# jxx2/MetaFEM.jl

Measured on AMD Instinct MI355X. Metric: DOF-updates/sec (assembly+CG iter) on 3D hex thermal conduction, higher is better.
Workload: dtype f64; 1 GPU; 3D thermal conduction, linear hex-8, 512x512x512 structured mesh (make_Brick): fused assembly (K + R) + 200 Jacobi-CG iterations per step; n_dof=135005697, nnz=3630961153, parallelism=single GPU

## Files before the change

include/metafem_mi355x_debug.h:

```cpp
#ifndef METAFEM_MI355X_DEBUG_H
#define METAFEM_MI355X_DEBUG_H

#include "metafem_mi355x.h"

#ifdef __cplusplus
extern "C" {
#endif

int64_t mfem_debug_sym_spmv_count(void);
long long mfem_debug_symp_fingerprint_count(void);
long long mfem_debug_symp_coded_count(void);
long long mfem_debug_symp_trim_count(void);
long long mfem_debug_symp_const_count(void);
long long mfem_debug_symp_const_steps(void);
int mfem_debug_spmv_scaled_layout(mfem_context ctx, mfem_csr A, const double* vals, const double* ssym, const double* x, double* y, double alpha, double beta,
                                  const double* dotw, double* partials_out , int32_t cap, int32_t* n_partials , int32_t* form );
int mfem_debug_set(const char* key, int64_t a, int64_t b);

int mfem_debug_lat27_cg_fused(void);
int64_t mfem_debug_lat27_pass1_bytes(mfem_csr A);
long long mfem_debug_lat27_spmv_count(void);
double mfem_debug_lat27_asymmetry(mfem_csr A);
long long mfem_debug_lat8_spmv_count(void);
double mfem_debug_lat8_asymmetry(mfem_csr A);
int mfem_debug_graph_comm_count(void);
long long mfem_debug_graph_launch_count(void);
int64_t mfem_debug_mesh_rows_count(void);
int64_t mfem_debug_mesh_direct_count(void);
int64_t mfem_debug_ws_bytes(mfem_context ctx);
int64_t mfem_debug_mesh_residual_count(void);
int64_t mfem_debug_mesh_operator_count(void);
int64_t mfem_debug_brick_operator_count(void);
int mfem_debug_brick_operator_apply_dot(mfem_context ctx, uint64_t op, const double* x, double* y, double alpha, double beta, const double* dotw,
                                        double* partials, int32_t* n_partials );
int64_t mfem_debug_mesh_ops_count(void);
int64_t mfem_debug_mesh_variants(int32_t reset);
int64_t mfem_debug_op_wave_count(int32_t kernel);
int64_t mfem_debug_sell_periodic_blocks(mfem_csr A);
int64_t mfem_debug_hex27_rows_count(void);
int64_t mfem_debug_hex27_mixed_count(void);
int64_t mfem_debug_hex27_direct_count(void);
int mfem_prof_spmv_enable(mfem_context ctx, int on);
int mfem_prof_spmv_read(mfem_context ctx, double* total_ms , int64_t* launches , int reset);
int mfem_prof_comm_enable(mfem_context ctx, int on);
int mfem_prof_comm_read(mfem_context ctx, double* halo_wait_ms , int64_t* halo_waits , double* allreduce_ms ,
                        int64_t* allreduces , int reset);
int mfem_debug_comm_selftest(mfem_context ctx, int64_t count, int32_t rounds);

unsigned long long mfem_debug_ws_address(mfem_context ctx);
long long mfem_debug_cg_ring_count(void);

int mfem_debug_ws_trial_log(mfem_context ctx, double* out4);

int mfem_debug_fail_host_alloc(int nth);


int mfem_debug_bsell_fields(mfem_csr A);
long long mfem_debug_bsell_spmv_count(void);
int mfem_debug_remainder_info(mfem_csr A, int64_t* rows , int64_t* entries , double* asym_before );
long long mfem_debug_rem_spmv_count(void);
int mfem_debug_csr_tplan(mfem_csr A, int64_t* bytes , double* build_ms );
int mfem_debug_brick_operator_signed_diagonal(mfem_context ctx, uint64_t op, double* d);
int mfem_debug_brick_multigrid_transfer(mfem_context ctx, uint64_t mg, int32_t level, int32_t restriction, const double* in, double* out);
double* mfem_debug_brick_multigrid_coords(uint64_t mg, int32_t level, int32_t dim_id);

#ifdef __cplusplus
}
#endif
#endif
```

metafem.jl_amd/_lib.py:

```python
from __future__ import annotations

import ctypes as C
import os

import torch

_HERE = os.path.dirname(os.path.abspath(__file__))
LIB_PATH = os.path.join(_HERE, "libmetafem_mi355x.so")


class MetaFEMError(RuntimeError):
    pass


def _load():
    if not os.path.exists(LIB_PATH):
        raise ImportError(
            f"{LIB_PATH} is missing: build it with `python -c 'import __graft_entry__ as g; g.build()'` "
            "(or `make -C metafem.jl_amd/csrc`).  There is no CPU fallback.")
    return C.CDLL(LIB_PATH, mode=C.RTLD_GLOBAL)


class _Lib:

    def __init__(self, cdll):
        object.__setattr__(self, "_cdll", cdll)

    def __getattr__(self, name):
        if name.startswith("mfem_debug_set_"):
            key = name[len("mfem_debug_set_"):]
            cdll = self._cdll

            def knob(a=0, b=0, _key=key):
                if _key == "recheck_scale":
                    return cdll.mfem_debug_set(b"recheck_scale_ppm", int(round(float(a) * 1e6)), 0)
                return cdll.mfem_debug_set(_key.encode(), int(a), int(b))
            return knob
        return getattr(self._cdll, name)


lib = _Lib(_load())

c_void_p, c_int, c_int32, c_int64, c_double, c_uint64, c_uint32 = (
    C.c_void_p, C.c_int, C.c_int32, C.c_int64, C.c_double, C.c_uint64, C.c_uint32)


class SolveOptions(C.Structure):
    _fields_ = [("method", c_int32), ("precond", c_int32), ("l_or_s", c_int32), ("maxiter", c_int32),
                ("max_pass", c_int32), ("check_every", c_int32), ("converge_tol", c_double), ("seed", c_uint64),
                ("fixed_iterations", c_int32), ("scale_in_place", c_int32), ("left_precond", c_int32),
                ("cg_variant", c_int32)]


class SolveStats(C.Structure):
    _fields_ = [("passes", c_int32), ("iterations", c_int32), ("final_res", c_double), ("initial_res", c_double),
                ("solve_ms", c_double), ("converged", c_int32), ("spmv_count", c_int32)]


class ThermalParams(C.Structure):
    _fields_ = [("k", c_double), ("h", c_double), ("Tenv", c_double), ("robin_faces", c_uint32), ("fixed_faces", c_uint32),
                ("h_penalty", c_double), ("Tw", c_double)]


class ElasticityParams(C.Structure):
    _fields_ = [("lam", c_double), ("mu", c_double), ("tau", c_double), ("penalty_faces", c_uint32),
                ("traction_faces", c_uint32), ("sig", c_double * 6)]


class KvalTerm(C.Structure):
    _fields_ = [("dual_sd", c_int32), ("base_sd", c_int32), ("block", c_int32), ("reserved", c_int32)]


class ResBatchTerm(C.Structure):
    _fields_ = [("dual_sd", c_int32), ("reserved", c_int32), ("cpID_shift", c_int64)]


class VarBatchTerm(C.Structure):
    _fields_ = [("sd", c_int32), ("reserved", c_int32), ("cpID_shift", c_int64), ("x", C.c_void_p)]


class ConstTerm(C.Structure):
    _fields_ = [("dual_sd", c_int32), ("base_sd", c_int32), ("block", c_int32), ("reserved", c_int32), ("coef", c_double)]


MAX_BATCH_TERMS = 48


class MeshDirectStats(C.Structure):
    _fields_ = [(n, c_int64) for n in ("batches", "tasks", "max_batch_doubles", "max_batch_elements", "geometry_evaluations", "device_bytes",
                                       "waves_per_trip", "max_control_point_doubles", "budget_doubles", "waves_per_workgroup", "lds_bytes",
                                       "split_owners", "max_batch_owners")]


class ResSymbol(C.Structure):
    _fields_ = [("word", c_int32), ("reserved", c_int32), ("shift", c_int64), ("x", C.c_void_p)]


class AffineTerm(C.Structure):
    _fields_ = [("dual_pos", c_int32), ("dual_sd", c_int32), ("n_pairs", c_int32), ("reserved", c_int32), ("c0", c_double),
                ("sym", c_int32 * 8), ("normal", c_int32 * 8), ("coef", c_double * 8)]


MAX_RES_SYMBOLS, MAX_RES_TERMS, MAX_RES_PAIRS = 16, 48, 8


class OperatorTerm(C.Structure):
    _fields_ = [("dual_sd", c_int32), ("base_sd", c_int32), ("block", c_int32), ("reserved", c_int32), ("coef", c_double),
                ("normal_coef", c_double * 3)]


MG_MAX_LEVELS = 12


class MultigridOptions(C.Structure):
    _fields_ = [("smoother_degree", c_int32), ("coarse_degree", c_int32), ("smoothing_range", c_double), ("coarse_range", c_double),
                ("eig_steps", c_int32), ("max_levels", c_int32)]


class MultigridInfo(C.Structure):
    _fields_ = [("levels", c_int32), ("sign", c_int32), ("nx", c_int32 * 12), ("ny", c_int32 * 12), ("nz", c_int32 * 12),
                ("lambda_max", c_double * 12), ("products", c_int64 * 12), ("setup_products", c_int64), ("bytes", c_int64), ("cycles", c_int64),
                ("setups", c_int64)]


ALLREDUCE_CB = C.CFUNCTYPE(c_int, c_void_p, C.POINTER(c_double), c_int32)
EXCHANGE_CB = C.CFUNCTYPE(c_int, c_void_p, C.POINTER(c_double), C.POINTER(c_double), C.POINTER(c_double), C.POINTER(c_double), c_int64)


class CommHostOps(C.Structure):
    _fields_ = [("user", c_void_p), ("allreduce_sum", ALLREDUCE_CB), ("neighbour_exchange", EXCHANGE_CB), ("flags", c_uint32),
                ("reserved", c_uint32)]


COMM_HOST_POISON_GHOSTS = 1


class OpLayout(C.Structure):
    _fields_ = [("itg", c_int32), ("itp", c_int32), ("n_sd", c_int32), ("n_host", c_int64), ("index_base", c_int32),
                ("n_colours", c_int32), ("colour_offsets", C.POINTER(c_int64))]


P = c_void_p
SIGNATURES = {
    "mfem_abi_version": (c_int, []),
    "mfem_last_error": (C.c_char_p, []),
    "mfem_context_create": (c_int, [c_int, P, C.POINTER(P)]),
    "mfem_context_set_stream": (c_int, [P, P]),
    "mfem_context_destroy": (c_int, [P]),
    "mfem_context_sync": (c_int, [P]),
    "mfem_csr_create": (c_int, [P, c_int64, c_int64, P, c_int, P, c_int, C.POINTER(P)]),
    "mfem_csr_destroy": (c_int, [P]),
    "mfem_spmv_csr": (c_int, [P, P, P, P, P, c_double, c_double]),
    "mfem_spmv_csr_t": (c_int, [P, P, P, P, P, c_double, c_double]),
    "mfem_axpby": (c_int, [P, c_int64, c_double, P, c_double, P]),
    "mfem_dot": (c_int, [P, c_int64, P, P, C.POINTER(c_double)]),
    "mfem_nrm2": (c_int, [P, c_int64, P, C.POINTER(c_double)]),
    "mfem_rand": (c_int, [P, c_int64, c_uint64, c_uint32, P]),
    "mfem_jacobi_by_diagonal": (c_int, [P, P, P, P]),
    "mfem_jacobi2_by_column": (c_int, [P, P, P, P]),
    "mfem_jacobi_by_row": (c_int, [P, P, P, P]),
    "mfem_mat_div_jacobi": (c_int, [P, P, P, P]),
    "mfem_debug_hex27_direct_count": (c_int64, []),
    "mfem_debug_hex27_mixed_count": (c_int64, []),
    "mfem_debug_hex27_rows_count": (c_int64, []),
    "mfem_debug_mesh_rows_count": (c_int64, []),
    "mfem_debug_mesh_variants": (c_int64, [c_int32]),
    "mfem_debug_op_wave_count": (c_int64, [c_int32]),
    "mfem_debug_bsell_fields": (c_int, [P]),
    "mfem_debug_bsell_spmv_count": (c_int64, []),
    "mfem_debug_sell_periodic_blocks": (c_int64, [P]),
    "mfem_debug_symp_fingerprint_count": (C.c_longlong, []),
    "mfem_debug_symp_coded_count": (C.c_longlong, []),
    "mfem_debug_symp_trim_count": (C.c_longlong, []),
    "mfem_debug_symp_const_count": (C.c_longlong, []),
    "mfem_debug_symp_const_steps": (C.c_longlong, []),
    "mfem_debug_spmv_scaled_layout": (c_int, [P, P, P, P, P, P, c_double, c_double, P, P, c_int32, C.POINTER(c_int32), C.POINTER(c_int32)]),
    "mfem_debug_set": (c_int, [C.c_char_p, c_int64, c_int64]),
    "mfem_debug_graph_comm_count": (c_int, []),
    "mfem_debug_graph_launch_count": (C.c_longlong, []),
    "mfem_debug_cg_ring_count": (C.c_longlong, []),
    "mfem_debug_lat27_cg_fused": (c_int, []),
    "mfem_debug_lat27_pass1_bytes": (c_int64, [P]),
    "mfem_prof_spmv_enable": (c_int, [P, c_int]),
    "mfem_prof_spmv_read": (c_int, [P, C.POINTER(c_double), C.POINTER(c_int64), c_int]),
    "mfem_prof_comm_enable": (c_int, [P, c_int]),
    "mfem_prof_comm_read": (c_int, [P, C.POINTER(c_double), C.POINTER(c_int64), C.POINTER(c_double), C.POINTER(c_int64), c_int]),
    "mfem_solve": (c_int, [P, P, P, P, P, C.POINTER(SolveOptions), C.POINTER(SolveStats)]),
    "mfem_solve_set_shadow": (c_int, [P, P, c_int32]),
    "mfem_brick_create": (c_int, [P, c_int32, c_int32, c_int32, c_double, c_double, c_double, c_int32, c_int32,
                                  C.POINTER(P)]),
    "mfem_brick_destroy": (c_int, [P]),
    "mfem_brick_num_controlpoints": (c_int64, [P]),
    "mfem_brick_num_elements": (c_int64, [P]),
    "mfem_brick_coords": (P, [P, c_int32]),
    "mfem_brick_set_slab": (c_int, [P, c_int32, c_int32]),
    "mfem_brick_pattern": (c_int, [P, P, c_int32, C.POINTER(P)]),
    "mfem_pattern_build": (c_int, [P, c_int32, c_int64, c_int64, P, c_int32, c_int32, C.POINTER(P), P]),
    "mfem_csr_rowptr64": (P, [P]),
    "mfem_csr_colidx": (P, [P]),
    "mfem_csr_nnz": (c_int64, [P]),
    "mfem_csr_n": (c_int64, [P]),
    "mfem_brick_assemble_thermal": (c_int, [P, P, P, C.POINTER(ThermalParams), P]),
    "mfem_brick_residual_thermal": (c_int, [P, P, C.POINTER(ThermalParams), P, P, P]),
    "mfem_brick_assemble_elasticity": (c_int, [P, P, P, C.POINTER(ElasticityParams), P]),
    "mfem_brick_residual_elasticity": (c_int, [P, P, C.POINTER(ElasticityParams), P, P]),
    "mfem_update_basic_elements": (c_int, [P, c_int32, c_int32, c_int32, c_int64, c_int64, P, P, P, P, c_int32, P, P]),
    "mfem_update_basic_boundary": (c_int, [P, c_int32, c_int32, c_int32, c_int32, c_int64, c_int64, P, P, P, P, P, P, P,
                                          c_int32, P, P, P]),
    "mfem_op_var": (c_int, [P, C.POINTER(OpLayout), P, c_int32, c_int64, P, P, P, P, P, c_int64]),
    "mfem_op_kval": (c_int, [P, C.POINTER(OpLayout), P, c_int32, c_int32, P, P, c_int64, P, P, P, c_int64]),
    "mfem_op_res": (c_int, [P, C.POINTER(OpLayout), P, c_int32, P, c_int64, P, P, P, P, c_int64]),
    "mfem_debug_lat27_spmv_count": (c_int64, []),
    "mfem_debug_lat27_asymmetry": (C.c_double, [c_void_p]),
    "mfem_debug_lat8_spmv_count": (c_int64, []),
    "mfem_debug_lat8_asymmetry": (C.c_double, [c_void_p]),
    "mfem_spmv_solver_layout": (c_int, [P, P, P, P, P, c_double, c_double]),
    "mfem_spmv_solver_layout_dot": (c_int, [P, P, P, P, P, c_double, c_double, C.POINTER(c_double)]),
    "mfem_csr_solver_layout": (c_int, [P, P, C.POINTER(c_int32), C.POINTER(c_int32), C.POINTER(c_int64), C.POINTER(c_int64)]),
    "mfem_csr_solver_layout_entries": (c_int, [P, P, C.POINTER(c_int64), C.POINTER(c_int32)]),
    "mfem_csr_solver_layout_bytes": (c_int, [P, P, C.POINTER(c_int64)]),
    "mfem_debug_sym_spmv_count": (c_int64, []),
    "mfem_op_kval_batch": (c_int, [P, C.POINTER(OpLayout), P, c_int32, C.POINTER(KvalTerm), P, P, c_int64, c_int64, P, P, P, c_int64]),
    "mfem_op_res_batch": (c_int, [P, C.POINTER(OpLayout), P, c_int32, C.POINTER(ResBatchTerm), P, P, P, P, P, c_int64]),
    "mfem_op_var_batch": (c_int, [P, C.POINTER(OpLayout), P, c_int32, C.POINTER(VarBatchTerm), P, P, P, P, c_int64]),
    "mfem_mesh_assemble_elements": (c_int, [P, c_int32, c_int32, c_int32, c_int64, c_int64, P, P, P, P, c_int32, c_int32,
                                            C.POINTER(ConstTerm), P, c_int64, P, P, c_int64, c_int32, C.POINTER(c_int64)]),
    "mfem_mesh_assemble_elements_rows": (c_int, [P, c_int32, c_int32, c_int32, c_int64, c_int64, P, P, P, P, c_int32, c_int32,
                                                 C.POINTER(ConstTerm), c_int32, P, P, P, P, P]),
    "mfem_mesh_assemble_elements_rows_set": (c_int, [P, c_int32, c_int32, c_int32, c_int64, c_int64, P, P, P, P, c_int32, c_int32,
                                                 C.POINTER(ConstTerm), c_int32, P, P, P, P, P]),
    "mfem_mesh_direct_plan_create": (c_int, [P, c_int32, c_int64, c_int64, c_int32, P, P, P, P, c_int32, P, C.POINTER(c_uint64)]),
    "mfem_mesh_direct_plan_destroy": (c_int, [c_uint64]),
    "mfem_mesh_direct_plan_stats": (c_int, [c_uint64, C.POINTER(MeshDirectStats)]),
    "mfem_mesh_assemble_elements_direct": (c_int, [P, c_int32, c_int32, c_int32, c_int64, c_int64, P, P, P, P, c_int32, c_int32,
                                                   C.POINTER(ConstTerm), c_int32, P, c_uint64, P, c_int32]),
    "mfem_debug_mesh_direct_count": (c_int64, []),
    "mfem_debug_ws_bytes": (c_int64, [P]),
    "mfem_mesh_row_ranks": (c_int, [P, c_int32, c_int64, c_int64, c_int32, P, P, P, P, c_int32, P]),
    "mfem_mesh_assemble_facets": (c_int, [P, c_int32, c_int32, c_int32, c_int32, c_int64, c_int64, P, P, P, P, P, P, P, c_int32,
                                          c_int32, C.POINTER(ConstTerm), P, c_int64, P, P, c_int64, c_int32, C.POINTER(c_int64)]),
    "mfem_mesh_residual_elements": (c_int, [P, c_int32, c_int32, c_int32, c_int64, c_int64, P, P, P, P, c_int32, c_int32,
                                            C.POINTER(ResSymbol), c_int32, C.POINTER(AffineTerm), P, P, P]),
    "mfem_mesh_residual_facets": (c_int, [P, c_int32, c_int32, c_int32, c_int32, c_int64, c_int64, P, P, P, P, P, P, P, c_int32,
                                          c_int32, C.POINTER(ResSymbol), c_int32, C.POINTER(AffineTerm), P, P, P]),
    "mfem_debug_mesh_residual_count": (c_int64, []),
    "mfem_mesh_operator_create": (c_int, [P, c_int32, c_int32, c_int64, c_int64, c_int32, P, P, c_int32, C.POINTER(c_uint64)]),
    "mfem_mesh_operator_set_elements": (c_int, [c_uint64, c_int32, P, P, P, P, c_int32, C.POINTER(OperatorTerm)]),
    "mfem_mesh_operator_add_facets": (c_int, [c_uint64, c_int32, c_int32, c_int64, P, P, P, P, P, P, P, c_int32, C.POINTER(OperatorTerm),
                                              C.POINTER(c_int32)]),
    "mfem_mesh_operator_set_terms": (c_int, [c_uint64, c_int32, c_int32, C.POINTER(OperatorTerm)]),
    "mfem_mesh_operator_set_variable_terms": (c_int, [c_uint64, c_int32, c_int32, C.POINTER(KvalTerm), P]),
    "mfem_mesh_operator_destroy": (c_int, [c_uint64]),
    "mfem_mesh_operator_apply": (c_int, [P, c_uint64, P, P, c_double, c_double]),
    "mfem_mesh_operator_diagonal": (c_int, [P, c_uint64, P]),
    "mfem_solve_operator": (c_int, [P, c_uint64, P, P, C.POINTER(SolveOptions), C.POINTER(SolveStats)]),
    "mfem_debug_mesh_operator_count": (c_int64, []),
    "mfem_brick_operator_create": (c_int, [P, P, C.POINTER(ThermalParams), C.POINTER(c_uint64)]),
    "mfem_brick_operator_set_params": (c_int, [c_uint64, C.POINTER(ThermalParams)]),
    "mfem_brick_operator_create_elasticity": (c_int, [P, P, C.POINTER(ElasticityParams), C.POINTER(c_uint64)]),
    "mfem_brick_operator_set_elasticity_params": (c_int, [c_uint64, C.POINTER(ElasticityParams)]),
    "mfem_brick_operator_create_hex27": (c_int, [P, P, C.POINTER(ThermalParams), C.POINTER(c_uint64)]),
    "mfem_brick_operator_destroy": (c_int, [c_uint64]),
    "mfem_brick_operator_apply": (c_int, [P, c_uint64, P, P, c_double, c_double]),
    "mfem_brick_operator_diagonal": (c_int, [P, c_uint64, P]),
    "mfem_debug_brick_operator_count": (c_int64, []),
    "mfem_debug_brick_operator_signed_diagonal": (c_int, [P, c_uint64, P]),
    "mfem_debug_brick_operator_apply_dot": (c_int, [P, c_uint64, P, P, c_double, c_double, P, P, C.POINTER(c_int32)]),
    "mfem_brick_multigrid_create": (c_int, [P, c_uint64, C.POINTER(MultigridOptions), C.POINTER(c_uint64)]),
    "mfem_brick_multigrid_create_elasticity": (c_int, [P, c_uint64, C.POINTER(MultigridOptions), C.POINTER(c_uint64)]),
    "mfem_brick_multigrid_create_hex27": (c_int, [P, c_uint64, C.POINTER(MultigridOptions), C.POINTER(c_uint64)]),
    "mfem_brick_multigrid_setup": (c_int, [P, c_uint64]),
    "mfem_brick_multigrid_apply": (c_int, [P, c_uint64, P, P]),
    "mfem_brick_multigrid_info": (c_int, [c_uint64, C.POINTER(MultigridInfo)]),
    "mfem_brick_multigrid_destroy": (c_int, [c_uint64]),
    "mfem_debug_brick_multigrid_transfer": (c_int, [P, c_uint64, c_int32, c_int32, P, P]),
    "mfem_debug_brick_multigrid_coords": (P, [c_uint64, c_int32, c_int32]),
    "mfem_mesh_var_elements": (c_int, [P, c_int32, c_int32, c_int32, c_int64, c_int64, P, P, P, P, c_int32, c_int32,
                                       C.POINTER(VarBatchTerm), P, P, c_int64]),
    "mfem_mesh_var_facets": (c_int, [P, c_int32, c_int32, c_int32, c_int32, c_int64, c_int64, P, P, P, P, P, P, P, c_int32,
                                     c_int32, C.POINTER(VarBatchTerm), P, P, P, c_int64]),
    "mfem_mesh_res_elements": (c_int, [P, c_int32, c_int32, c_int32, c_int64, c_int64, P, P, P, P, c_int32, c_int32,
                                       C.POINTER(ResBatchTerm), P, P, P, P, P]),
    "mfem_mesh_res_facets": (c_int, [P, c_int32, c_int32, c_int32, c_int32, c_int64, c_int64, P, P, P, P, P, P, P, c_int32,
                                     c_int32, C.POINTER(ResBatchTerm), P, P, P, P, P]),
    "mfem_mesh_kval_elements": (c_int, [P, c_int32, c_int32, c_int32, c_int64, c_int64, P, P, P, P, c_int32, c_int32,
                                        C.POINTER(KvalTerm), P, P, c_int64, P, P, c_int64, c_int32, C.POINTER(c_int64)]),
    "mfem_mesh_kval_elements_rows": (c_int, [P, c_int32, c_int32, c_int32, c_int64, c_int64, P, P, P, P, c_int32, c_int32,
                                             C.POINTER(KvalTerm), P, P, c_int32, P, P, P, P, P]),
    "mfem_mesh_kval_facets": (c_int, [P, c_int32, c_int32, c_int32, c_int32, c_int64, c_int64, P, P, P, P, P, P, P, c_int32,
                                      c_int32, C.POINTER(KvalTerm), P, P, c_int64, P, P, c_int64, c_int32, C.POINTER(c_int64)]),
    "mfem_debug_mesh_ops_count": (c_int64, []),
    "mfem_comm_unique_id": (c_int, [P]),
    "mfem_comm_create": (c_int, [P, c_int32, c_int32, P, C.POINTER(P)]),
    "mfem_comm_destroy": (c_int, [P]),
    "mfem_context_set_comm": (c_int, [P, P, c_int64, c_int64, c_int32]),
    "mfem_allreduce_sum": (c_int, [P, P, c_int32]),
    "mfem_halo_exchange": (c_int, [P, P]),
    "mfem_halo_reduce": (c_int, [P, P]),
    "mfem_comm_create_host": (c_int, [P, c_int32, c_int32, C.POINTER(CommHostOps), C.POINTER(P)]),
    "mfem_csr_ncols": (c_int64, [P]),
    "mfem_csr_replan": (c_int, [P, P]),
    "mfem_csr_spmv_bytes": (c_int, [P, P, C.POINTER(c_int64), C.POINTER(c_int64)]),
    "mfem_debug_comm_selftest": (c_int, [P, c_int64, c_int32]),
    "mfem_debug_ws_address": (C.c_ulonglong, [P]),
    "mfem_debug_fail_host_alloc": (c_int, [c_int]),
    "mfem_debug_ws_trial_log": (c_int, [P, C.POINTER(C.c_double)]),
    "mfem_debug_remainder_info": (c_int, [P, C.POINTER(c_int64), C.POINTER(c_int64), C.POINTER(C.c_double)]),
    "mfem_debug_rem_spmv_count": (C.c_longlong, []),
    "mfem_debug_csr_tplan": (c_int, [P, C.POINTER(c_int64), C.POINTER(C.c_double)]),
}

for _name, (_res, _args) in SIGNATURES.items():
    _fn = getattr(lib, _name)
    _fn.restype = _res
    _fn.argtypes = _args


def check(rc: int) -> None:
    if rc != 0:
        raise MetaFEMError(f"libmetafem_mi355x rc={rc}: {lib.mfem_last_error().decode()}")
```

metafem.jl_amd/csrc/api.hip:

```cpp
#include <stdarg.h>
#include <atomic>

#include <exception>
#include <mutex>
#include <new>
#include <set>

#include "common.h"
#include <string>

static std::mutex g_ctx_mutex;
static std::set<mfem_context_s*> g_live_contexts;
bool mfem_context_alive(mfem_context_s* ctx) {
  std::lock_guard<std::mutex> lk(g_ctx_mutex);
  return g_live_contexts.count(ctx) != 0;
}

static thread_local char g_err[1024] = "";

void mfem_set_error(const char* fmt, ...) {
  va_list ap;
  va_start(ap, fmt);
  vsnprintf(g_err, sizeof(g_err), fmt, ap);
  va_end(ap);
}

int mfem_api_exception(const char* entry) noexcept {
  try {
    throw;
  } catch (const std::bad_alloc&) {
    mfem_set_error("%s: host memory exhausted (std::bad_alloc)", entry);
    return MFEM_ERR_ALLOC;
  } catch (const std::exception& e) {
    mfem_set_error("%s: internal error: %s", entry, e.what());
    return MFEM_ERR_INTERNAL;
  } catch (...) {
    mfem_set_error("%s: internal error (unknown C++ exception)", entry);
    return MFEM_ERR_INTERNAL;
  }
}

static std::atomic<int> g_fail_host_alloc{0};
extern "C" int mfem_debug_fail_host_alloc(int nth) try {
  g_fail_host_alloc.store(nth > 0 ? nth : 0);
  return MFEM_OK;
} MFEM_API_CATCH("mfem_debug_fail_host_alloc")
void mfem_host_alloc_probe() {
  int v = g_fail_host_alloc.load();
  while (v > 0) {
    if (g_fail_host_alloc.compare_exchange_weak(v, v - 1)) {
      if (v == 1) throw std::bad_alloc();
      return;
    }
  }
}

std::atomic<int> mfem_debug_epoch{0};

extern "C" int mfem_abi_version(void) { return MFEM_ABI_VERSION; }
extern "C" const char* mfem_last_error(void) { return g_err; }

int mfem_ws_release(void* raw);
static int context_allocate(mfem_context_s* c) {
  MFEM_CHECK_HIP(hipMalloc(&c->d_partials, sizeof(double) * MFEM_MAX_PARTIALS * 8));
  MFEM_CHECK_HIP(hipMalloc(&c->d_scalars, sizeof(double) * MFEM_NSCALARS));
  MFEM_CHECK_HIP(hipHostMalloc(&c->h_scalars, sizeof(double) * MFEM_NSCALARS));
  MFEM_CHECK_HIP(hipMalloc(&c->d_flags, sizeof(int32_t) * MFEM_NFLAGS));
  MFEM_CHECK_HIP(hipHostMalloc(&c->h_flags, sizeof(int32_t) * MFEM_NFLAGS));
  MFEM_CHECK_HIP(hipMemsetAsync(c->d_scalars, 0, sizeof(double) * MFEM_NSCALARS, c->stream));
  MFEM_CHECK_HIP(hipMemsetAsync(c->d_flags, 0, sizeof(int32_t) * MFEM_NFLAGS, c->stream));
  MFEM_CHECK_HIP(hipEventCreate(&c->ev0));
  MFEM_CHECK_HIP(hipEventCreate(&c->ev1));
  return MFEM_OK;
}

static void context_release(mfem_context_s* ctx) {
  if (ctx->d_partials) hipFree(ctx->d_partials);
  if (ctx->d_scalars) hipFree(ctx->d_scalars);
  if (ctx->h_scalars) hipHostFree(ctx->h_scalars);
  if (ctx->d_flags) hipFree(ctx->d_flags);
  if (ctx->h_flags) hipHostFree(ctx->h_flags);
  (void)mfem_ws_release(ctx->ws_raw);
  (void)mfem_ws_release(ctx->ws_alt_raw);
  if (ctx->prof_ev) {
    for (int i = 0; i < 2 * MFEM_PROF_PAIRS; ++i)
      if (ctx->prof_ev[i]) hipEventDestroy(ctx->prof_ev[i]);
    delete[] ctx->prof_ev;
  }
  if (ctx->ev0) hipEventDestroy(ctx->ev0);
  if (ctx->ev1) hipEventDestroy(ctx->ev1);
  for (int i = 0; i < MFEM_GRAPH_SLOTS; ++i)
    if (ctx->graph_exec[i]) hipGraphExecDestroy(ctx->graph_exec[i]);
  if (ctx->graph_ev) hipEventDestroy(ctx->graph_ev);
  if (ctx->graph_stream) hipStreamDestroy(ctx->graph_stream);
}

extern "C" int mfem_context_create(int device, void* stream, mfem_context* out) try {
  MFEM_REQUIRE(out != nullptr, "out is null");
  int ndev = 0;
  MFEM_CHECK_HIP(hipGetDeviceCount(&ndev));
  MFEM_REQUIRE(device >= 0 && device < ndev, "no such HIP device");
  MFEM_CHECK_HIP(hipSetDevice(device));
  hipDeviceProp_t prop;
  MFEM_CHECK_HIP(hipGetDeviceProperties(&prop, device));
  if (strncmp(prop.gcnArchName, "gfx950", 6) != 0) {
    mfem_set_error("libmetafem_mi355x is built for gfx950 only, device %d is %s", device, prop.gcnArchName);
    return MFEM_ERR_UNSUPPORTED;
  }
  mfem_host_alloc_probe();
  mfem_context_s* c = new mfem_context_s();
  memset(c, 0, sizeof(*c));
  c->device = device;
  c->stream = (hipStream_t)stream;
  c->num_cus = prop.multiProcessorCount;
  int rc = context_allocate(c);
  if (rc != MFEM_OK) {
    context_release(c);
    delete c;
    return rc;
  }
  {
    std::lock_guard<std::mutex> lk(g_ctx_mutex);
    g_live_contexts.insert(c);
  }
  *out = c;
  return MFEM_OK;
} MFEM_API_CATCH("mfem_context_create")

extern "C" int mfem_context_set_stream(mfem_context ctx, void* stream) try {
  MFEM_REQUIRE(ctx != nullptr, "ctx is null");
  ctx->stream = (hipStream_t)stream;
  return MFEM_OK;
} MFEM_API_CATCH("mfem_context_set_stream")

extern "C" int mfem_context_sync(mfem_context ctx) try {
  MFEM_REQUIRE(ctx != nullptr, "ctx is null");
  MFEM_CHECK_HIP(hipStreamSynchronize(ctx->stream));
  return MFEM_OK;
} MFEM_API_CATCH("mfem_context_sync")

extern "C" int mfem_context_destroy(mfem_context ctx) try {
  if (!ctx) return MFEM_OK;
  {
    std::lock_guard<std::mutex> lk(g_ctx_mutex);
    g_live_contexts.erase(ctx);
  }
  hipStreamSynchronize(ctx->stream);
  context_release(ctx);
  delete ctx;
  return MFEM_OK;
} MFEM_API_CATCH("mfem_context_destroy")

int mfem_prof_flush(mfem_context_s* ctx) {
  if (ctx->prof_used == 0) return MFEM_OK;
  MFEM_CHECK_HIP(hipEventSynchronize(ctx->prof_ev[2 * ctx->prof_used - 1]));
  for (int k = 0; k < ctx->prof_used; ++k) {
    float ms = 0.f;
    MFEM_CHECK_HIP(hipEventElapsedTime(&ms, ctx->prof_ev[2 * k], ctx->prof_ev[2 * k + 1]));
    ctx->prof_ms += ms;
  }
  ctx->prof_count += ctx->prof_used;
  ctx->prof_used = 0;
  return MFEM_OK;
}

extern "C" int mfem_prof_spmv_enable(mfem_context ctx, int on) try {
  MFEM_REQUIRE(ctx, "null ctx");
  if (on && !ctx->prof_ev) {
    ctx->prof_ev = new hipEvent_t[2 * MFEM_PROF_PAIRS]();
    for (int i = 0; i < 2 * MFEM_PROF_PAIRS; ++i) MFEM_CHECK_HIP(hipEventCreate(&ctx->prof_ev[i]));
  }
  if (!on) {
    int rc = mfem_prof_flush(ctx);
    if (rc) return rc;
  }
  ctx->prof_on = on ? 1 : 0;
  return MFEM_OK;
} MFEM_API_CATCH("mfem_prof_spmv_enable")

extern "C" int mfem_prof_spmv_read(mfem_context ctx, double* total_ms, int64_t* launches, int reset) try {
  MFEM_REQUIRE(ctx && total_ms && launches, "null argument");
  int rc = mfem_prof_flush(ctx);
  if (rc) return rc;
  *total_ms = ctx->prof_ms;
  *launches = ctx->prof_count;
  if (reset) {
    ctx->prof_ms = 0.0;
    ctx->prof_count = 0;
  }
  return MFEM_OK;
} MFEM_API_CATCH("mfem_prof_spmv_read")

uint64_t mfem_next_csr_serial() {
  static std::atomic<uint64_t> next{1};
  return next.fetch_add(1);
}

void mfem_graphs_invalidate(mfem_context_s* ctx) {
  for (int i = 0; i < MFEM_GRAPH_SLOTS; ++i)
    if (ctx->graph_exec[i]) {
      hipGraphExecDestroy(ctx->graph_exec[i]);
      ctx->graph_exec[i] = nullptr;
      ctx->graph_key[i] = 0;
    }
}

static std::atomic<size_t> g_ws_align{0}, g_ws_offset{0};
extern "C" int mfem_debug_set_ws_placement(long long align, long long offset) try {
  g_ws_align = align > 0 ? (size_t)align : 0;
  g_ws_offset = offset > 0 ? (size_t)offset : 0;
  return MFEM_OK;
} MFEM_API_CATCH("mfem_debug_set_ws_placement")
static int ws_alloc(mfem_context_s* ctx, void** raw, size_t bytes) {
  (void)ctx;
  *raw = nullptr;
  MFEM_CHECK_HIP(hipMalloc(raw, bytes));
  return MFEM_OK;
}
static int ws_free(void* raw) {
  if (raw) MFEM_CHECK_HIP(hipFree(raw));
  return MFEM_OK;
}
int mfem_ws_release(void* raw) { return ws_free(raw); }
extern "C" int64_t mfem_debug_ws_bytes(mfem_context ctx) { return ctx ? (int64_t)ctx->ws_bytes : 0; }
extern "C" unsigned long long mfem_debug_ws_address(mfem_context ctx) { return ctx ? (unsigned long long)(uintptr_t)ctx->ws : 0ull; }
#include <chrono>
static double now_ms() { return std::chrono::duration<double, std::milli>(std::chrono::steady_clock::now().time_since_epoch()).count(); }
int mfem_ws_next_candidate(mfem_context_s* ctx) {
  const bool verbose = getenv("MFEM_WS_TRIAL_VERBOSE") != nullptr;
  double t0 = now_ms();
  MFEM_CHECK_HIP(hipStreamSynchronize(ctx->stream));
  if (verbose) fprintf(stderr, "ws trial: sync %.1f ms\n", now_ms() - t0);
  const size_t need = ctx->ws_bytes + g_ws_align + g_ws_offset;
  if (ctx->ws_alt_raw) {
    t0 = now_ms();
    {
      int rcf = ws_free(ctx->ws_raw);
      if (rcf) return rcf;
    }
    if (verbose) fprintf(stderr, "ws trial: free %.1f ms\n", now_ms() - t0);
    ctx->ws = ctx->ws_raw = nullptr;
  }
  size_t freeb = 0, totalb = 0;
  void* raw = nullptr;
  bool ok = hipMemGetInfo(&freeb, &totalb) == hipSuccess && freeb >= need + ((size_t)4 << 30);
  t0 = now_ms();
  if (ok && ws_alloc(ctx, &raw, need) != MFEM_OK) ok = false;
  if (verbose) fprintf(stderr, "ws trial: alloc %.1f ms\n", now_ms() - t0);
  if (!ok) {
    (void)hipGetLastError();
    if (!ctx->ws_raw) {
      ctx->ws = ctx->ws_alt;
      ctx->ws_raw = ctx->ws_alt_raw;
      ctx->ws_alt = ctx->ws_alt_raw = nullptr;
    }
    return MFEM_OK;
  }
  if (ctx->ws_raw) {
    ctx->ws_alt = ctx->ws;
    ctx->ws_alt_raw = ctx->ws_raw;
  }
  ctx->ws_raw = raw;
  uintptr_t p = (uintptr_t)raw;
  if (g_ws_align) p = (p + g_ws_align - 1) / g_ws_align * g_ws_align;
  ctx->ws = (void*)(p + g_ws_offset);
  ctx->ws_try += 1;
  return MFEM_OK;
}
int mfem_ws_decide(mfem_context_s* ctx, bool keep_current) {
  MFEM_CHECK_HIP(hipStreamSynchronize(ctx->stream));
  if (ctx->ws_alt_raw) {
    if (keep_current) {
      int rcf = ws_free(ctx->ws_alt_raw);
      if (rcf) return rcf;
    } else {
      int rcf = ws_free(ctx->ws_raw);
      if (rcf) return rcf;
      ctx->ws = ctx->ws_alt;
      ctx->ws_raw = ctx->ws_alt_raw;
    }
  }
  ctx->ws_alt = ctx->ws_alt_raw = nullptr;
  ctx->ws_try = 99;
  return MFEM_OK;
}
int mfem_ws_reserve(mfem_context_s* ctx, size_t bytes) {
  if (bytes <= ctx->ws_bytes) return MFEM_OK;
  MFEM_CHECK_HIP(hipStreamSynchronize(ctx->stream));
  int rcf = ws_free(ctx->ws_raw);
  if (!rcf) rcf = ws_free(ctx->ws_alt_raw);
  ctx->ws = ctx->ws_raw = ctx->ws_alt = ctx->ws_alt_raw = nullptr;
  ctx->ws_try = 0;
  ctx->ws_bytes = 0;
  if (rcf) return rcf;
  rcf = ws_alloc(ctx, &ctx->ws_raw, bytes + g_ws_align + g_ws_offset);
  if (rcf) return rcf;
  uintptr_t p = (uintptr_t)ctx->ws_raw;
  if (g_ws_align) p = (p + g_ws_align - 1) / g_ws_align * g_ws_align;
  ctx->ws = (void*)(p + g_ws_offset);
  ctx->ws_bytes = bytes;
  return MFEM_OK;
}

extern "C" {
int mfem_debug_set_spmv(int, int);
int mfem_debug_set_ell(int);
int mfem_debug_set_sell(int);
int mfem_debug_set_lat27(int);
int mfem_debug_set_lat8(int);
int mfem_debug_set_layout_min_rows(int64_t, int64_t);
int mfem_debug_set_graphs(int, int64_t);
int mfem_debug_set_idrs(int);
int mfem_debug_set_bicgstabl(int);
int mfem_debug_set_gmres(int);
int mfem_debug_set_vec_grid(int);
int mfem_debug_set_halo_overlap(int);
int mfem_debug_set_hex27(int);
int mfem_debug_set_elasticity(int);
int mfem_debug_set_hex8_thermal(int);
int mfem_debug_set_ws_placement(long long, long long);
int mfem_debug_set_ws_trial(int);
int mfem_debug_set_cg_streaming(int);
int mfem_debug_set_cg_ring(int);
int mfem_debug_set_cg_single_max_rows(int64_t);
int mfem_debug_set_csr_strips(int, int64_t);
int mfem_debug_set_remainder(int);
int mfem_debug_set_recheck_scale(double);
int mfem_debug_set_bsell(int);
}
extern int g_mesh_gather_rows, g_mesh_abl, g_mesh_stage_min_itp, g_mesh_term_matrix;
extern int g_op_wave_forms, g_op_wave_min_itp;
extern int64_t g_mesh_direct_budget;
extern "C" int mfem_debug_set(const char* key, int64_t a, int64_t b) try {
  MFEM_REQUIRE(key, "null key");
  const std::string k(key);
  if (k == "spmv") return mfem_debug_set_spmv((int)a, (int)b);
  if (k == "ell") return mfem_debug_set_ell((int)a);
  if (k == "sell") return mfem_debug_set_sell((int)a);
  if (k == "lat27") return mfem_debug_set_lat27((int)a);
  if (k == "lat8") return mfem_debug_set_lat8((int)a);
  if (k == "layout_min_rows") return mfem_debug_set_layout_min_rows(a, b);
  if (k == "graphs") return mfem_debug_set_graphs((int)a, b);
  if (k == "idrs") return mfem_debug_set_idrs((int)a);
  if (k == "bicgstabl") return mfem_debug_set_bicgstabl((int)a);
  if (k == "gmres") return mfem_debug_set_gmres((int)a);
  if (k == "vec_grid") return mfem_debug_set_vec_grid((int)a);
  if (k == "halo_overlap") return mfem_debug_set_halo_overlap((int)a);
  if (k == "hex27") return mfem_debug_set_hex27((int)a);
  if (k == "elasticity") return mfem_debug_set_elasticity((int)a);
  if (k == "hex8_thermal") return mfem_debug_set_hex8_thermal((int)a);
  if (k == "ws_placement") return mfem_debug_set_ws_placement((long long)a, (long long)b);
  if (k == "ws_trial") return mfem_debug_set_ws_trial((int)a);
  if (k == "cg_streaming") return mfem_debug_set_cg_streaming((int)a);
  if (k == "cg_ring") return mfem_debug_set_cg_ring((int)a);
  if (k == "cg_single_max_rows") return mfem_debug_set_cg_single_max_rows(a);
  if (k == "csr_strips") return mfem_debug_set_csr_strips((int)a, b);
  if (k == "remainder") return mfem_debug_set_remainder((int)a);
  if (k == "mesh_gather_rows") { g_mesh_gather_rows = (int)a; return MFEM_OK; }
  if (k == "bsell") return mfem_debug_set_bsell((int)a);
  if (k == "op_wave_forms") { g_op_wave_forms = (int)a; g_op_wave_min_itp = b > 0 ? (int)b : 10; return MFEM_OK; }
  if (k == "mesh_stage_min_itp") { g_mesh_stage_min_itp = a > 0 ? (int)a : 16; return MFEM_OK; }
  if (k == "mesh_term_matrix") { g_mesh_term_matrix = (int)a; return MFEM_OK; }
  if (k == "mesh_direct_budget") { g_mesh_direct_budget = a > 0 ? a : 0; return MFEM_OK; }
  if (k == "mesh_abl") { g_mesh_abl = (int)a; return MFEM_OK; }
  if (k == "recheck_scale_ppm") return mfem_debug_set_recheck_scale((double)a * 1e-6);
  mfem_set_error("mfem_debug_set: unknown key '%s'", key);
  return MFEM_ERR_INVALID;
} MFEM_API_CATCH("mfem_debug_set")
```

metafem.jl_amd/csrc/common.h:

```cpp
#pragma once
#include <hip/hip_runtime.h>
#include <atomic>
#include <mutex>
#include <unordered_map>
#include <stdint.h>
#include <stdio.h>
#include <string.h>

#if defined(__HIP_DEVICE_COMPILE__) && !defined(__gfx950__)
#error "metafem_mi355x is written for gfx950 (MI355X) only: counted s_waitcnt vmcnt(k) pipelines assume loads and stores share one in-order counter, global_load_lds_dwordx4 and v_mfma_f64 are used directly -- build with --offload-arch=gfx950"
#endif
#include "../../include/metafem_mi355x.h"
#include "../../include/metafem_mi355x_debug.h"
#include "csr_decide.h"
#include "sell_decide.h"
#include "lat_decide.h"

#define MFEM_WAVE 64
#define MFEM_BLOCK 256
#define MFEM_MAX_PARTIALS 4096
static_assert(LAT_MAX_GATHER_GRID == MFEM_MAX_PARTIALS, "a workgroup of the tiles' gather pass writes one partial sum");
#define MFEM_NFLAGS 80
#define MFEM_NSCALARS 4096

void mfem_set_error(const char* fmt, ...);

int mfem_api_exception(const char* entry) noexcept;
#define MFEM_API_CATCH(entry) catch (...) { return mfem_api_exception(entry); }
void mfem_host_alloc_probe();

#define MFEM_CHECK_HIP(expr)                                                                  \
  do {                                                                                        \
    hipError_t _e = (expr);                                                                   \
    if (_e != hipSuccess) {                                                                   \
      mfem_set_error("%s:%d: %s -> %s", __FILE__, __LINE__, #expr, hipGetErrorString(_e));    \
      return MFEM_ERR_HIP;                                                                    \
    }                                                                                         \
  } while (0)

#define MFEM_REQUIRE(cond, msg)                                      \
  do {                                                               \
    if (!(cond)) {                                                   \
      mfem_set_error("%s:%d: %s (%s)", __FILE__, __LINE__, msg, #cond); \
      return MFEM_ERR_INVALID;                                       \
    }                                                                \
  } while (0)

#define MFEM_CHECK_LAUNCH() MFEM_CHECK_HIP(hipGetLastError())

template <typename T> struct __attribute__((visibility("hidden"))) DevBuf {
  T* p = nullptr;
  DevBuf() = default;
  DevBuf(DevBuf&& o) noexcept : p(o.release()) {}
  DevBuf& operator=(DevBuf&& o) noexcept { if (this != &o) { reset(); p = o.release(); } return *this; }
  DevBuf(const DevBuf&) = delete;
  DevBuf& operator=(const DevBuf&) = delete;
  ~DevBuf() { reset(); }
  hipError_t alloc(size_t count) { reset(); return hipMalloc((void**)&p, sizeof(T) * count); }
  void reset() { if (p) (void)hipFree(p); p = nullptr; }
  T* release() { T* q = p; p = nullptr; return q; }
  operator T*() const { return p; }
};

struct mfem_comm_s;

#define MFEM_MAX_ZONES 8
struct SpmvPart {
  int part;
  int nz;
  int64_t lo[MFEM_MAX_ZONES], hi[MFEM_MAX_ZONES];
};
__host__ __device__ __forceinline__ bool spmv_part_skip(const SpmvPart& P, int64_t r0, int64_t r1) {
  if (P.part == 0) return false;
  bool bnd = false;
  for (int z = 0; z < P.nz; ++z) bnd = bnd || (r0 < P.hi[z] && r1 > P.lo[z]);
  return P.part == 1 ? bnd : !bnd;
}


#define MFEM_GRAPH_SLOTS 4
struct mfem_context_s {
  int device;
  hipStream_t stream;
  int num_cus;
  double* d_partials;
  double* d_scalars;
  double* h_scalars;
  int32_t* d_flags;
  int32_t* h_flags;
  void* ws;
  void* ws_raw;
  size_t ws_bytes;
  int ws_try;
  void* ws_alt;
  void* ws_alt_raw;
  float ws_try_ms;
  float ws_log[4];
  const double* shadow;
  int32_t shadow_count;
  mfem_comm_s* comm;
  int64_t halo_plane_len;
  int32_t halo_fields;
  hipEvent_t ev0, ev1;
  int prof_on;
  int prof_used;
  hipEvent_t* prof_ev;
  double prof_ms;
  int64_t prof_count;
  hipGraphExec_t graph_exec[MFEM_GRAPH_SLOTS];
  uint64_t graph_key[MFEM_GRAPH_SLOTS];
  int graph_next;
  hipStream_t graph_stream;
  hipEvent_t graph_ev;
  int graph_active;
  int force_csr;
  int probe_active;
};
#define MFEM_PROF_PAIRS 1024
int mfem_prof_flush(mfem_context_s* ctx);

struct mfem_operator_head;
struct mfem_csr_s {
  mfem_context_s* ctx;
  uint64_t serial;
  int64_t n, nnz;
  const void* rowptr;
  int rowptr_bits;
  const int32_t* colidx;
  int index_base;
  int32_t max_row_nnz;
  CsrPlan plan;
  int nb_F, nb_checked;
  int64_t rb_ntiles;
  int64_t rb_elided;
  int32_t* rb_rows;
  uint8_t* cw_elide;
  int32_t lat_m1, lat_m2, lat_fields;
  int32_t lat_m0, lat_plo, lat_gw;
  int32_t lat_inferred;
  uint16_t* diag_off;
  void* owned_rowptr;
  void* owned_colidx;
  int64_t x_offset;
  int64_t ncols;
  int ell_state, ell_K;
  int64_t ell_npad;
  int32_t* ell_cols;
  const double* ell_src;
  double* ell_vals;
  int dia_state, dia_classes;
  void* dia_dev;
  int32_t* dia_flags;
  int32_t dia_regular_blocks;
  int dia_triples;
  int sym_state;
  int64_t sym_c0, sym_c1;
  int sym_cls;
  int sym_S;
  int64_t sym_mx, sym_myz;
  int ell_bound_mode;
  int dia_kernel;
  int symp_state;
  int symp_m1, symp_m2;
  int64_t symp_PL;
  int symp_p0, symp_p1;
  int symp_NS, symp_NPk;
  int symp_B;
  int symp_trim;
  int symp_DC;
  int symp_dneg;
  int symp_CS;
  int symp_cs_last;
  int64_t symp_flagged, symp_flagged_last;
  double symp_cst[27];
  int symp_ccode;
  int symp_dc_last;
  double* symp_vals;
  SellLayout sell;
  LatTiles lat27, lat8;
  int lat_refused;
  int rem_active;
  int64_t rem_nrows, rem_nent, rem_cap_rows, rem_cap_ent;
  int32_t* rem_rows;
  int64_t* rem_ptr;
  int32_t* rem_len;
  int32_t* rem_col;
  double* rem_val;
  unsigned long long* rem_cnt;
  void* rem_sort_tmp;
  size_t rem_sort_bytes;
  double rem_asym_before;
  int64_t rem_last_rows, rem_last_ent;
  struct mfem_tplan_s* tplan;
  struct mfem_operator_head* op;
  double* op_scratch;
  const double* op_dsc;
  uint64_t op_epoch;
};
struct mfem_tplan_s {
  mfem_csr_s* AT;
  void* perm;
  int perm_bits;
  double* vals;
  int64_t bytes;
  double build_ms;
};
static inline CsrShape mfem_csr_shape(const mfem_csr_s* A) { return {A->n, A->nnz, A->max_row_nnz}; }
template <typename F> static inline auto mfem_by_rowptr(const mfem_csr_s* A, F&& f) { return A->rowptr_bits == 64 ? f(int64_t{}) : f(int32_t{}); }
int mfem_tplan_get(mfem_context_s* ctx, mfem_csr_s* A, mfem_tplan_s** out);
void mfem_tplan_free(mfem_csr_s* A);
int mfem_tplan_gather(mfem_context_s* ctx, const mfem_tplan_s* P, const double* src, double* valsT, const double* d1, const double* d2);
bool mfem_rem_enabled();
bool mfem_rem_diag();
void mfem_rem_clear(mfem_csr_s* A);
void mfem_rem_free(mfem_csr_s* A);
int mfem_rem_build(mfem_context_s* ctx, mfem_csr_s* A, const double* vals, int n_fields, const double* y1, const double* y2, const double* scale,
                   double gate, bool* built);
int mfem_rem_apply(mfem_context_s* ctx, mfem_csr_s* A, const double* x, const double* dsc, double* y, double alpha, const double* dotw,
                   double* partials, int* n_partials, const int32_t* done_flag);
int64_t mfem_rem_design_bytes(const mfem_csr_s* A);
int mfem_spmv_lat8_launch(mfem_context_s* ctx, mfem_csr_s* A, const double* vals, const double* x, double* y, double alpha, double beta,
                          const double* dotw, double* partials, int* n_partials, const int32_t* done_flag, int part);
int64_t mfem_lat8_design_bytes(const mfem_csr_s* A);
int64_t mfem_lat8_entries(const mfem_csr_s* A);
int mfem_lattice_hint_from_row0(mfem_context_s* ctx, mfem_csr_s* A);
static inline LatShape mfem_lat_shape(const mfem_csr_s* A, int64_t min_rows) {
  return {A->n, A->ncols, A->max_row_nnz, A->lat_m0, A->lat_m1, A->lat_m2, A->lat_fields, A->lat_plo, A->lat_gw, min_rows};
}
static inline void mfem_lat_unbind(mfem_csr_s* A, LatTiles& T) {
  if (T.vals) A->rem_active = 0;
  T.vals = T.dump = nullptr;
  T.src = T.dsc = nullptr;
}
int mfem_sym_probe(mfem_context_s* ctx, mfem_csr_s* A, LatTiles* T, const double* vals, double* scratch, double amax, double* asym, int rem_fields);
int mfem_spmv_lat27_launch(mfem_context_s* ctx, mfem_csr_s* A, const double* vals, const double* x, double* y, double alpha,
                           double beta, const double* dotw, double* partials, int* n_partials, const int32_t* done_flag, int part);
int64_t mfem_lat27_design_bytes(const mfem_csr_s* A);
int64_t mfem_lat27_entries(const mfem_csr_s* A);
int mfem_node_block_fields(mfem_context_s* ctx, mfem_csr_s* A);
int mfem_spmv_sell_launch(mfem_context_s* ctx, mfem_csr_s* A, const double* vals, const double* x, double* y, double alpha,
                          double beta, const double* dotw, double* partials, int* n_partials, const int32_t* done_flag, int part);
int mfem_ell_diag(mfem_context_s* ctx, mfem_csr_s* A, double* d);
int mfem_spmv_ell_launch(mfem_context_s* ctx, mfem_csr_s* A, const double* vals, const double* x, double* y, double alpha,
                         double beta, const double* dotw, double* partials, int* n_partials, const int32_t* done_flag,
                         const SpmvPart& part);
struct SpmvArgs {
  const double* x; double* y; double alpha, beta; const double* dotw; double* partials; int* n_partials; const int32_t* done_flag; const SpmvPart& part;
};
__attribute__((visibility("hidden"))) int mfem_spmv_csr_launch(mfem_context_s* ctx, mfem_csr_s* A, const double* vals, const double* x, double* y, double alpha,
                                                             double beta, const double* dotw, double* partials, int* n_partials, const int32_t* done_flag,
                                                             const SpmvPart& part);
__attribute__((visibility("hidden"))) CsrKnobs mfem_csr_knobs();

enum mfem_layout : int32_t { MFEM_LAYOUT_CSR = 0, MFEM_LAYOUT_ELL = 1, MFEM_LAYOUT_DIA = 2, MFEM_LAYOUT_SELL = 3, MFEM_LAYOUT_LAT27 = 4, MFEM_LAYOUT_LAT8 = 5,
                             MFEM_LAYOUT_OPERATOR = 6  };
struct mfem_layout_plan_s {
  mfem_layout tile, rows;
  size_t tile_bytes, rows_bytes;
};
int mfem_layout_plan(mfem_context_s* ctx, mfem_csr_s* A, bool is_cg, bool allow_tiles, mfem_layout_plan_s* P);
int mfem_layout_bind(mfem_context_s* ctx, mfem_csr_s* A, mfem_layout mode, const double* vals, double* buf, const double* dsc, const double* ssym,
                     double* scratch, bool allow_rem);
mfem_layout mfem_layout_bound(const mfem_csr_s* A, const double* vals);
void mfem_layout_unbind(mfem_csr_s* A);
void mfem_layout_drop(mfem_csr_s* A);

int mfem_ws_reserve(mfem_context_s* ctx, size_t bytes);
int mfem_ws_next_candidate(mfem_context_s* ctx);
int mfem_ws_decide(mfem_context_s* ctx, bool keep_current);
uint64_t mfem_next_csr_serial();
bool mfem_context_alive(mfem_context_s* ctx);
void mfem_graphs_invalidate(mfem_context_s* ctx);
extern std::atomic<int> mfem_debug_epoch;

__device__ __forceinline__ double wave_reduce_sum(double v) {
#pragma unroll
  for (int off = 32; off > 0; off >>= 1) v += __shfl_down(v, off, MFEM_WAVE);
  return v;
}

__device__ __forceinline__ void mfem_lds_barrier() { asm volatile("s_waitcnt lgkmcnt(0)\n\ts_barrier" ::: "memory"); }

__device__ __forceinline__ bool mfem_xcd_tile(int tcount, int& tsub) {
  const int chunk = (tcount + 7) >> 3;
  tsub = (int)(blockIdx.x & 7) * chunk + (int)(blockIdx.x >> 3);
  return !((int)(blockIdx.x >> 3) >= chunk || tsub >= tcount);
}

__device__ __forceinline__ double block_reduce_sum(double v, double* smem ) {
  v = wave_reduce_sum(v);
  const int lane = threadIdx.x & 63, w = threadIdx.x >> 6;
  __syncthreads();
  if (lane == 0) smem[w] = v;
  __syncthreads();
  double r = 0.0;
  if (threadIdx.x == 0) {
    const int nw = (blockDim.x + 63) >> 6;
    for (int i = 0; i < nw; ++i) r += smem[i];
  }
  __syncthreads();
  return r;
}

static inline int mfem_resident_per_cu(const void* kernel, int block_threads, size_t dyn_lds, int fallback) {
  static std::mutex mu;
  static std::unordered_map<const void*, int> cache;
  std::lock_guard<std::mutex> lk(mu);
  auto it = cache.find(kernel);
  if (it != cache.end()) return it->second;
  int occ = 0;
  const hipError_t e = hipOccupancyMaxActiveBlocksPerMultiprocessor(&occ, kernel, block_threads, dyn_lds);
  const int v = (e == hipSuccess && occ >= 1) ? occ : fallback;
  cache[kernel] = v;
  return v;
}
static inline int mfem_grid_for(int64_t work_items, int per_block, int cap) {
  int64_t g = (work_items + per_block - 1) / per_block;
  if (g < 1) g = 1;
  if (g > cap) g = cap;
  return (int)g;
}
```

metafem.jl_amd/csrc/krylov.h:

```cpp
#pragma once
#include "blas1.h"

#define MFEM_MAX_S 32

enum {
  S_RZ0 = 0, S_RZ1 = 1, S_RR = 2, S_PAP = 3, S_TMP0 = 4, S_TMP1 = 5, S_TMP2 = 6, S_TMP3 = 7,
  S_SOLVER = 16
};
enum { F_DONE = 0, F_ITER = 1, F_SPMV = 2, F_AUX = 3 };

__device__ __forceinline__ double mfem_recip_nr(double d) {
  double y = __builtin_amdgcn_rcp(d);
  double e = fma(-d, y, 1.0);
  y = fma(y, e, y);
  e = fma(-d, y, 1.0);
  return fma(y, e, y);
}

struct LatCgUpdate {
  int32_t zrec, cur;
  const double* sw;
  double smax2, gate2, n_inv;
  const double* dinv;
  double* r;
  const double* S;
  const int32_t* flags;
  double* partials2;
  const double* pap_partials;
  int32_t np;
};
bool mfem_lat27_cg_fused(const mfem_context_s* ctx, const mfem_csr_s* A, const double* vals);
const double* mfem_lat27_dot_partials(const mfem_csr_s* A, int* np);
int mfem_lat27_gather_cg_update(mfem_context_s* ctx, mfem_csr_s* A, const LatCgUpdate& U, int grid);

struct KrylovVecs {
  int64_t n, nv;
  double* x;
  double* b;
  double* d;
  const double* dinv;
  const double* cg_s = nullptr;
  double cg_smax = 1.0, cg_smin = 1.0;
  double* w[3 * MFEM_MAX_S + 8];
  int nwork;
  int cg_ring = 1;
  bool x_zero = false;
  double* gm = nullptr;
  mfem_csr_s* AT = nullptr;
  double* valsT = nullptr;
};

int mfem_fill(mfem_context_s* ctx, int64_t n, double v, double* x);
int mfem_sum_partials(mfem_context_s* ctx, const double* partials, int np, double* d_out);
int mfem_true_residual(mfem_context_s* ctx, mfem_csr_s* A, const double* vals, const double* b, const double* x,
                       double* r, double* d_rr);
int mfem_pass_residual(mfem_context_s* ctx, mfem_csr_s* A, const double* vals, const KrylovVecs& V, double* r, double* d_rr, int* spmv_out);
int mfem_read_scalars(mfem_context_s* ctx, int first, int count);
int mfem_read_flags(mfem_context_s* ctx);
typedef int mfem_pass_fn(mfem_context_s* ctx, mfem_csr_s* A, const double* vals, KrylovVecs& V, const mfem_solve_options* o, int s, double tol,
                         int64_t n_global, int* iters_out, int* spmv_out);
mfem_pass_fn mfem_cg_pass, mfem_cg_single_pass, mfem_bicgstabl_pass, mfem_cgs2_pass, mfem_idrs_pass, mfem_gmres_pass;
mfem_pass_fn mfem_cgs_pass, mfem_tfqmr_pass, mfem_lsqr_pass;
mfem_pass_fn mfem_cg_mg_pass;
size_t mfem_gmres_workspace_bytes();
int mfem_cg_ring_depth(int64_t nv);

inline uint64_t mfem_hash_bytes(uint64_t h, const void* data, size_t bytes) {
  const unsigned char* p = (const unsigned char*)data;
  for (size_t i = 0; i < bytes; ++i) h = (h ^ p[i]) * 1099511628211ull;
  return h;
}
template <typename T>
inline uint64_t mfem_hash(uint64_t h, const T& v) { return mfem_hash_bytes(h, &v, sizeof(T)); }
#define MFEM_HASH_SEED 1469598103934665603ull

inline uint64_t mfem_csr_graph_key(uint64_t key, const mfem_csr_s* A) {
  key = mfem_hash(key, A->serial); key = mfem_hash(key, A->rowptr); key = mfem_hash(key, A->colidx);
  key = mfem_hash(key, A->n); key = mfem_hash(key, A->nnz); key = mfem_hash(key, A->max_row_nnz);
  key = mfem_hash(key, A->index_base); key = mfem_hash(key, A->ell_vals);
  key = mfem_hash(key, A->ell_bound_mode + 16 * A->dia_kernel); key = mfem_hash(key, A->sell.vals); key = mfem_hash(key, A->lat27.vals); key = mfem_hash(key, A->lat8.vals); key = mfem_hash(key, A->symp_vals);
  key = mfem_hash(key, A->symp_B + 16 * A->symp_DC + 32 * A->symp_dneg + 64 * A->symp_trim);
  key = mfem_hash(key, A->symp_CS);
  if (A->symp_CS) { key = mfem_hash_bytes(key, A->symp_cst, sizeof(A->symp_cst)); key = mfem_hash(key, A->symp_ccode); }
  key = mfem_hash(key, A->lat27.dsc); key = mfem_hash(key, A->lat8.dsc);
  key = mfem_hash(key, A->rem_active);
  key = mfem_hash(key, A->op != nullptr); key = mfem_hash(key, A->op_epoch); key = mfem_hash(key, A->op_scratch); key = mfem_hash(key, A->op_dsc);
  if (A->rem_active) { key = mfem_hash(key, A->rem_nrows); key = mfem_hash(key, A->rem_rows); key = mfem_hash(key, A->rem_col); key = mfem_hash(key, A->rem_val); }
  key = mfem_hash(key, mfem_debug_epoch.load());
  return key;
}

inline uint64_t mfem_pass_key(int method, const mfem_csr_s* A, const double* vals, const KrylovVecs& V, double tol, int64_t n_global,
                              const mfem_solve_options* o) {
  uint64_t key = mfem_hash(MFEM_HASH_SEED, method);
  key = mfem_csr_graph_key(key, A); key = mfem_hash(key, vals); key = mfem_hash(key, V.w[0]); key = mfem_hash(key, V.x);
  key = mfem_hash(key, V.b); key = mfem_hash(key, V.nv); key = mfem_hash(key, tol); key = mfem_hash(key, n_global);
  key = mfem_hash(key, o->maxiter); key = mfem_hash(key, o->fixed_iterations);
  return key;
}

extern std::atomic<int> mfem_graph_comm_broken;
extern std::atomic<long long> mfem_graph_comm_captures;
extern std::atomic<long long> mfem_graph_launches;
template <class Body>
inline int mfem_cycle_run(mfem_context_s* ctx, uint64_t key, Body body) {
  if (!ctx->graph_active) return body();
  for (int i = 0; i < MFEM_GRAPH_SLOTS; ++i)
    if (ctx->graph_exec[i] && ctx->graph_key[i] == key) {
      ++mfem_graph_launches;
      MFEM_CHECK_HIP(hipGraphLaunch(ctx->graph_exec[i], ctx->stream));
      return MFEM_OK;
    }
  const int slot = ctx->graph_next;
  ctx->graph_next = (slot + 1) % MFEM_GRAPH_SLOTS;
  if (ctx->graph_exec[slot]) {
    hipGraphExecDestroy(ctx->graph_exec[slot]);
    ctx->graph_exec[slot] = nullptr;
  }
  MFEM_CHECK_HIP(hipStreamBeginCapture(ctx->stream, hipStreamCaptureModeThreadLocal));
  const int rc = body();
  hipGraph_t g = nullptr;
  const hipError_t e = hipStreamEndCapture(ctx->stream, &g);
  auto comm_fallback = [&](const char* what, hipError_t err) -> int {
    (void)hipGetLastError();
    mfem_graph_comm_broken = 1;
    ctx->graph_active = 0;
    fprintf(stderr, "metafem_mi355x: %s failed with a communicator attached (%s): cycles run as direct launches from now on\n", what, hipGetErrorString(err));
    return body();
  };
  if (rc) {
    if (g) hipGraphDestroy(g);
    if (ctx->comm && e != hipSuccess) return comm_fallback("capturing a Krylov cycle", e);
    return rc;
  }
  if (e != hipSuccess || !g) {
    if (ctx->comm) return comm_fallback("hipStreamEndCapture", e);
    mfem_set_error("hipStreamEndCapture: %s", hipGetErrorString(e));
    return MFEM_ERR_HIP;
  }
  hipGraphExec_t exec = nullptr;
  const hipError_t ei = hipGraphInstantiate(&exec, g, nullptr, nullptr, 0);
  hipGraphDestroy(g);
  if (ei != hipSuccess) {
    if (ctx->comm) return comm_fallback("hipGraphInstantiate", ei);
    mfem_set_error("hipGraphInstantiate: %s", hipGetErrorString(ei));
    return MFEM_ERR_HIP;
  }
  if (ctx->comm) ++mfem_graph_comm_captures;
  ctx->graph_exec[slot] = exec;
  ctx->graph_key[slot] = key;
  ++mfem_graph_launches;
  MFEM_CHECK_HIP(hipGraphLaunch(exec, ctx->stream));
  return MFEM_OK;
}
```

metafem.jl_amd/csrc/spmv_ell.h:

```cpp
#pragma once
#include <vector>

#include "layouts.h"
#include "spmv_symp.h"
#include "symp_trim_decide.h"
#include "symp_const_decide.h"

#define ELL_B 128
__host__ __device__ __forceinline__ int64_t ell_base(int64_t r, int K) { return (r >> 7) * ((int64_t)K * ELL_B) + (r & (ELL_B - 1)); }

typedef double e_d2 __attribute__((ext_vector_type(2)));
typedef int e_i2 __attribute__((ext_vector_type(2)));
typedef double u_d2 __attribute__((ext_vector_type(2), aligned(8)));

#define DIA_MAXD 96
#define DIA_MAXC 4
struct DiaOffsets {
  int ncls;
  int D[DIA_MAXC];
  int32_t off[DIA_MAXC][DIA_MAXD];
};

struct SympGeom {
  int64_t PL, nx;
  int m1, m2, p0, p1, NS, NPk;
  int nseg;
  int B, NR;
  int DC;
  long long unit;
  int ms1, ms2;
  int rim_pp;
  int64_t rim_rows, rim_units;
};
struct SympConst {
  double v[27];
  int32_t code, valid;
};
#define SPC_COUNT_AT 20
#define SPC_REF_AT 22
static_assert(SPC_REF_AT % 2 == 0 && SPC_REF_AT * 4 + sizeof(SympConst) <= MFEM_NFLAGS * 4, "the reference row must fit the context's flags");
struct SympTail {
  int on, K;
  int rim;
  int64_t n, npad, lo, hi;
  const DiaOffsets* Op;
  const int32_t* flags;
  const int32_t* cols;
  const double* ell;
};

#if defined(DV_ABL) && DV_ABL == 1
#define DIA_ST(p, v) do { if ((v) == 1.2345e300) __builtin_nontemporal_store((v), (p)); } while (0)
#elif defined(DV_ABL) && DV_ABL == 3
#define DIA_ST(p, v) (*(p) = (v))
#else
#define DIA_ST(p, v) __builtin_nontemporal_store((v), (p))
#endif
#define SYM_LD(p) __builtin_nontemporal_load(p)

template <int RPT, int U, bool TRIPLES>
__device__ __forceinline__ void dia_rows(int64_t r, int64_t n, int64_t npad, int K, const DiaOffsets& O,
                                         const int32_t* __restrict__ flags, const int32_t* __restrict__ cols,
                                         const double* __restrict__ vals, const double* __restrict__ x, double* __restrict__ y,
                                         double alpha, double beta, const double* __restrict__ dotw, int xcd, double& dot_acc,
                                         int64_t skip_lo = 0, int64_t skip_hi = 0) {
  constexpr int H = RPT / 2;
  const double* v = vals + ell_base(r, K);
  e_d2 acc[H];
  double xself0 = 0.0, xself1 = 0.0;
  bool have_self = false;
#pragma unroll
  for (int h = 0; h < H; ++h) acc[h] = (e_d2){0.0, 0.0};
  const int64_t blk = r / (64 * RPT) * (RPT / 2);
  const int cls = __builtin_amdgcn_readfirstlane(flags[blk]) - 1;
  bool interior = cls >= 0;
  if (RPT == 4) interior = interior && ((blk + 1) * 128 < npad) && flags[blk + 1] == cls + 1;
  const int32_t* off = O.off[cls < 0 ? 0 : cls];
  const int D = O.D[cls < 0 ? 0 : cls];
  if (interior && TRIPLES && RPT == 2) {
    for (int s = 0; s < D; s += 3) {
      const e_d2 va = __builtin_nontemporal_load(reinterpret_cast<const e_d2*>(v + s * ELL_B));
      const e_d2 vb = __builtin_nontemporal_load(reinterpret_cast<const e_d2*>(v + (s + 1) * ELL_B));
      const e_d2 vc = __builtin_nontemporal_load(reinterpret_cast<const e_d2*>(v + (s + 2) * ELL_B));
      const u_d2* xp = reinterpret_cast<const u_d2*>(x + r + off[s]);
      const u_d2 xa = xp[0], xb = xp[1];
      acc[0].x += va.x != 0.0 ? va.x * xa.x : 0.0;
      acc[0].y += va.y != 0.0 ? va.y * xa.y : 0.0;
      acc[0].x += vb.x != 0.0 ? vb.x * xa.y : 0.0;
      acc[0].y += vb.y != 0.0 ? vb.y * xb.x : 0.0;
      acc[0].x += vc.x != 0.0 ? vc.x * xb.x : 0.0;
      acc[0].y += vc.y != 0.0 ? vc.y * xb.y : 0.0;
      if (off[s + 1] == 0) {
        xself0 = xa.y;
        xself1 = xb.x;
        have_self = true;
      }
    }
  } else if (interior) {
    int s = 0;
    for (; s + U <= D; s += U) {
      e_d2 vv[U][H];
      u_d2 xx[U][H];
#pragma unroll
      for (int u = 0; u < U; ++u)
#pragma unroll
        for (int h = 0; h < H; ++h) {
          vv[u][h] = __builtin_nontemporal_load(reinterpret_cast<const e_d2*>(v + (s + u) * ELL_B) + h);
          xx[u][h] = *(reinterpret_cast<const u_d2*>(x + r + off[s + u]) + h);
        }
#pragma unroll
      for (int u = 0; u < U; ++u)
#pragma unroll
        for (int h = 0; h < H; ++h) {
          acc[h].x += vv[u][h].x != 0.0 ? vv[u][h].x * xx[u][h].x : 0.0;
          acc[h].y += vv[u][h].y != 0.0 ? vv[u][h].y * xx[u][h].y : 0.0;
        }
    }
    for (; s < D; ++s)
#pragma unroll
      for (int h = 0; h < H; ++h) {
        const e_d2 vv = __builtin_nontemporal_load(reinterpret_cast<const e_d2*>(v + s * ELL_B) + h);
        const u_d2 xx = *(reinterpret_cast<const u_d2*>(x + r + off[s]) + h);
        acc[h].x += vv.x != 0.0 ? vv.x * xx.x : 0.0;
        acc[h].y += vv.y != 0.0 ? vv.y * xx.y : 0.0;
      }
  } else {
    const int32_t* c = cols + ell_base(r, K);
    for (int s = 0; s < K; ++s)
#pragma unroll
      for (int h = 0; h < H; ++h) {
        if (r + 2 * h >= npad) continue;
        const e_d2 vv = __builtin_nontemporal_load(reinterpret_cast<const e_d2*>(v + s * ELL_B) + h);
        const e_i2 cc = __builtin_nontemporal_load(reinterpret_cast<const e_i2*>(c + s * ELL_B) + h);
        acc[h].x += vv.x * x[cc.x];
        acc[h].y += vv.y * x[cc.y];
      }
  }
#pragma unroll
  for (int h = 0; h < H; ++h) {
    const int64_t rr = r + 2 * h;
    if (rr >= n) break;
    double y0 = alpha * acc[h].x, y1 = alpha * acc[h].y;
    const bool one = rr < skip_lo || rr >= skip_hi;
    const bool two = rr + 1 < n && (rr + 1 < skip_lo || rr + 1 >= skip_hi);
    if (beta != 0.0) {
      if (one) y0 += beta * y[rr];
      if (two) y1 += beta * y[rr + 1];
    }
    if (one) y[rr] = y0;
    if (two) y[rr + 1] = y1;
    if (dotw) {
      if (RPT == 2 && have_self && dotw == x) {
        if (one) dot_acc += y0 * xself0;
        if (two) dot_acc += y1 * xself1;
      } else {
        if (one) dot_acc += y0 * dotw[rr];
        if (two) dot_acc += y1 * dotw[rr + 1];
      }
    }
  }
}

struct EllKnobs {
  std::atomic<int> enable{1};
  std::atomic<int> dia{1};
  std::atomic<int> symp_trim{0};
  std::atomic<int> symp_const{0};
  std::atomic<int> grid_mult{6};
  std::atomic<int> shared_x{1};
  std::atomic<int> xcd{0};
  std::atomic<int> symp_coded{1};
  std::atomic<int> sym{1};
  std::atomic<int> symp{1};
  std::atomic<int> symp_bands{0};
  std::atomic<int> symp_tail{1};
  std::atomic<int> symp_direct{1};
  std::atomic<int> dia_pipe{1};
  std::atomic<int> dia_fast{1};
  std::atomic<int> symp_fingerprint{1};
};
extern EllKnobs g_ell;
extern std::atomic<int64_t> g_layout_min_rows_dia, g_layout_min_rows_cols;

enum DiaKernel : int { DIA_NONE = 0, DIA_ROWS, DIA_ROWS_TRIPLES, DIA_SYM27, DIA_SYMP };
DiaKernel mfem_dia_kernel_wanted(const mfem_csr_s* A, DiaKernel refused = DIA_NONE, bool* direct = nullptr);
int mfem_dia_plan(mfem_context_s* ctx, mfem_csr_s* A);
int mfem_dia_copy(mfem_context_s* ctx, mfem_csr_s* A, const double* vals, double* buf, const double* dsc, const double* ssym, const SympGeom& G,
                  double* pvals, double* rim, bool want_fp, bool* fp_made, unsigned char* sflags = nullptr, bool* flags_made = nullptr);
int mfem_dia_launch(mfem_context_s* ctx, mfem_csr_s* A, bool triples, int cap, const SpmvArgs& a);
int mfem_dia_launch_outside(mfem_context_s* ctx, mfem_csr_s* A, const SpmvArgs& a, double* partials, int64_t lo, int64_t hi, int* ngrid);
void mfem_sym_plan(mfem_csr_s* A, const int32_t* off, int lc, int64_t m2, int64_t PL, int64_t run_lo, int64_t run_hi);
bool mfem_sym_wanted(const mfem_csr_s* A, DiaKernel k);
SympGeom mfem_symp_geom(const mfem_context_s* ctx, const mfem_csr_s* A);
int64_t mfem_symp_steps(const mfem_csr_s* A, int B = 0, int trim = -1);
int mfem_symp_bands_wanted(const mfem_csr_s* A);
int mfem_symp_bands(const mfem_csr_s* A);
int mfem_symp_trim_wanted(const mfem_csr_s* A);
int mfem_symp_trim(const mfem_csr_s* A);
int64_t mfem_symp_copy_doubles(const mfem_csr_s* A, int B, int trim);
int64_t mfem_symp_swept_rows(const mfem_csr_s* A);
int mfem_symp_coded_wanted(DiaKernel k, bool fast, const double* ssym);
int mfem_symp_coded(const mfem_csr_s* A);
bool mfem_dia_fill_fast(const mfem_csr_s* A, const double* dsc, bool direct);
int64_t mfem_sym_entries(const mfem_context_s* ctx, const mfem_csr_s* A, DiaKernel k);
int mfem_sym_verdict(mfem_context_s* ctx, mfem_csr_s* A, DiaKernel k, const double* buf, double* pvals, const SympGeom& G, bool direct, bool fp_made, bool* ok,
                     bool* dc_refused, int* dneg, bool flags_made = false, SympConst* cst = nullptr, int64_t* flagged = nullptr);
unsigned char* mfem_symp_flags_of(double* pvals, const SympGeom& G);
int mfem_sym_launch(mfem_context_s* ctx, mfem_csr_s* A, DiaKernel k, const SpmvArgs& a);
```

metafem.jl_amd/csrc/spmv_ell.hip:

```cpp
#include "blas1.h"
#include "spmv_ell.h"

std::atomic<int64_t> g_layout_min_rows_dia{262144};
std::atomic<int64_t> g_layout_min_rows_cols{1000000};
#define LAT27_MIN_ROWS 180000
std::atomic<int64_t> g_layout_min_rows_lat27{LAT27_MIN_ROWS};
extern "C" int mfem_debug_set_layout_min_rows(int64_t diagonal_slots, int64_t explicit_columns) try {
  ++mfem_debug_epoch;
  g_layout_min_rows_dia = diagonal_slots;
  g_layout_min_rows_cols = explicit_columns;
  g_layout_min_rows_lat27 = explicit_columns < LAT27_MIN_ROWS ? explicit_columns : LAT27_MIN_ROWS;
  return MFEM_OK;
} MFEM_API_CATCH("mfem_debug_set_layout_min_rows")

EllKnobs g_ell;
extern "C" int mfem_debug_set_ell(int enable) try {
  ++mfem_debug_epoch;
  g_ell.enable = enable & 1;
  g_ell.dia = (enable & 2) ? 0 : 1;
  g_ell.symp_trim = (enable & 4) ? 2 : (enable & 8) ? 1 : 0;
  g_ell.symp_const = (enable & 16) ? 2 : (enable & 32) ? 1 : 0;
  if ((enable >> 8) & 255) g_ell.grid_mult = (enable >> 8) & 255;
  g_ell.shared_x = ((enable >> 16) & 15) == 8 ? 0 : 1;
  g_ell.xcd = (enable >> 20) & 1;
  g_ell.symp_coded = ((enable >> 21) & 1) ? 0 : 1;
  g_ell.sym = ((enable >> 22) & 1) ? 0 : 1;
  g_ell.symp = ((enable >> 23) & 1) ? 0 : 1;
  g_ell.symp_bands = ((enable >> 24) & 1) ? 1 : ((enable >> 25) & 1) ? 2 : 0;
  g_ell.symp_tail = ((enable >> 26) & 1) ? 0 : 1;
  g_ell.symp_direct = ((enable >> 27) & 1) ? 0 : 1;
  g_ell.dia_pipe = ((enable >> 28) & 1) ? 0 : 1;
  g_ell.dia_fast = ((enable >> 29) & 1) ? 0 : 1;
  g_ell.symp_fingerprint = ((enable >> 30) & 1) ? 0 : 1;
  return MFEM_OK;
} MFEM_API_CATCH("mfem_debug_set_ell")

template <typename RP>
__global__ __launch_bounds__(MFEM_BLOCK) void k_ell_cols(int64_t n, int64_t npad, int K, const RP* __restrict__ rowptr,
                                                           const int32_t* __restrict__ col, int base, int32_t* __restrict__ out) {
  const int64_t stride = (int64_t)gridDim.x * blockDim.x;
  for (int64_t r = blockIdx.x * (int64_t)blockDim.x + threadIdx.x; r < npad; r += stride) {
    int64_t lo = 0;
    int len = 0;
    if (r < n) {
      lo = (int64_t)rowptr[r] - base;
      len = (int)((int64_t)rowptr[r + 1] - base - lo);
    }
    const int32_t self = (int32_t)(r < n ? r : 0);
    for (int s = 0; s < K; ++s) out[ell_base(r, K) + s * ELL_B] = s < len ? col[lo + s] - base : self;
  }
}

template <typename RP>
__global__ __launch_bounds__(MFEM_BLOCK) void k_ell_vals_lds(int64_t n, int64_t npad, int K, const RP* __restrict__ rowptr,
                                                               const double* __restrict__ vals, int base, double* __restrict__ out,
                                                               const int32_t* __restrict__ col, const double* __restrict__ dsc) {
  extern __shared__ double lds[];
  const int lane = threadIdx.x & 63, w = threadIdx.x >> 6, nw = blockDim.x >> 6;
  double* T = lds + (size_t)w * 64 * K;
  const int64_t ntiles = npad >> 6;
  for (int64_t tile = (int64_t)blockIdx.x * nw + w; tile < ntiles; tile += (int64_t)gridDim.x * nw) {
    const int64_t r0 = tile << 6, r = r0 + lane;
    const int64_t rend = (r0 + 64 < n) ? r0 + 64 : n;
    int64_t lo = 0;
    int len = 0;
    if (r < n) {
      lo = (int64_t)rowptr[r] - base;
      len = (int)((int64_t)rowptr[r + 1] - base - lo);
    }
    const int64_t s0 = r0 < n ? (int64_t)rowptr[r0] - base : 0;
    const int cnt = r0 < n ? (int)((int64_t)rowptr[rend] - base - s0) : 0;
    constexpr int NB = 28;
    for (int i0 = lane; i0 < cnt; i0 += 64 * NB) {
      double tv[NB];
#pragma unroll
      for (int u = 0; u < NB; ++u) {
        const int i = i0 + 64 * u;
        tv[u] = i < cnt ? vals[s0 + i] : 0.0;
        if (dsc && i < cnt) tv[u] /= dsc[col[s0 + i] - base];
      }
#pragma unroll
      for (int u = 0; u < NB; ++u) {
        const int i = i0 + 64 * u;
        if (i < cnt) T[i] = tv[u];
      }
    }
    __builtin_amdgcn_wave_barrier();
    __builtin_amdgcn_s_waitcnt(0xC07F);
    const int off = (int)(lo - s0);
    for (int s = 0; s < K; ++s) out[ell_base(r, K) + s * ELL_B] = s < len ? T[off + s] : 0.0;
    __builtin_amdgcn_wave_barrier();
  }
}

template <int RPT, int U>
__global__ __launch_bounds__(MFEM_BLOCK) void k_spmv_ell(int64_t n, int64_t npad, int K, const int32_t* __restrict__ cols,
                                                           const double* __restrict__ vals, const double* __restrict__ x,
                                                           double* __restrict__ y, double alpha, double beta,
                                                           const double* __restrict__ dotw, double* __restrict__ partials,
                                                           const int32_t* __restrict__ done_flag, SpmvPart part) {
  __shared__ double red[4];
  if (done_flag && done_flag[0]) return;
  double dot_acc = 0.0;
  const int64_t stride = (int64_t)gridDim.x * blockDim.x * RPT;
  for (int64_t r = (blockIdx.x * (int64_t)blockDim.x + threadIdx.x) * RPT; r < n; r += stride) {
    if (spmv_part_skip(part, r, r + RPT)) continue;
    const double* v = vals + ell_base(r, K);
    const int32_t* c = cols + ell_base(r, K);
    if (RPT == 1) {
      double acc = 0.0;
      int s = 0;
      for (; s + U <= K; s += U) {
        double vv[U];
        int32_t cc[U];
#pragma unroll
        for (int u = 0; u < U; ++u) {
          vv[u] = __builtin_nontemporal_load(v + (s + u) * ELL_B);
          cc[u] = __builtin_nontemporal_load(c + (s + u) * ELL_B);
        }
#pragma unroll
        for (int u = 0; u < U; ++u) acc += vv[u] * x[cc[u]];
      }
      for (; s < K; ++s) acc += __builtin_nontemporal_load(v + s * ELL_B) * x[__builtin_nontemporal_load(c + s * ELL_B)];
      double yv = alpha * acc;
      if (beta != 0.0) yv += beta * y[r];
      y[r] = yv;
      if (dotw) dot_acc += yv * dotw[r];
    } else {
      e_d2 acc = {0.0, 0.0};
      int s = 0;
      for (; s + U <= K; s += U) {
        e_d2 vv[U];
        e_i2 cc[U];
#pragma unroll
        for (int u = 0; u < U; ++u) {
          vv[u] = __builtin_nontemporal_load(reinterpret_cast<const e_d2*>(v + (s + u) * ELL_B));
          cc[u] = __builtin_nontemporal_load(reinterpret_cast<const e_i2*>(c + (s + u) * ELL_B));
        }
#pragma unroll
        for (int u = 0; u < U; ++u) {
          acc.x += vv[u].x * x[cc[u].x];
          acc.y += vv[u].y * x[cc[u].y];
        }
      }
      for (; s < K; ++s) {
        const e_d2 v1 = __builtin_nontemporal_load(reinterpret_cast<const e_d2*>(v + s * ELL_B));
        const e_i2 c1 = __builtin_nontemporal_load(reinterpret_cast<const e_i2*>(c + s * ELL_B));
        acc.x += v1.x * x[c1.x];
        acc.y += v1.y * x[c1.y];
      }
      double y0 = alpha * acc.x, y1 = alpha * acc.y;
      const bool two = r + 1 < n;
      if (beta != 0.0) {
        y0 += beta * y[r];
        if (two) y1 += beta * y[r + 1];
      }
      y[r] = y0;
      if (two) y[r + 1] = y1;
      if (dotw) {
        dot_acc += y0 * dotw[r];
        if (two) dot_acc += y1 * dotw[r + 1];
      }
    }
  }
  if (partials) {
    const double b = block_reduce_sum(dot_acc, red);
    if (threadIdx.x == 0) partials[blockIdx.x] = b;
  }
}

__global__ __launch_bounds__(MFEM_BLOCK) void k_ell_diag(int64_t n, int K, const DiaOffsets* __restrict__ Op,
                                                           const int32_t* __restrict__ flags, const int32_t* __restrict__ cols,
                                                           const double* __restrict__ vals, double* __restrict__ d) {
  const int64_t stride = (int64_t)gridDim.x * blockDim.x;
  for (int64_t r = blockIdx.x * (int64_t)blockDim.x + threadIdx.x; r < n; r += stride) {
    const int64_t b = ell_base(r, K);
    const int cls = flags ? flags[r >> 7] - 1 : -1;
    double out = 1.0;
    if (cls >= 0) {
      const int D = Op->D[cls];
      for (int s = 0; s < D; ++s)
        if (Op->off[cls][s] == 0) {
          const double v = vals[b + s * ELL_B];
          if (v != 0.0) out = fabs(v);
          break;
        }
    } else {
      for (int s = 0; s < K; ++s)
        if (cols[b + s * ELL_B] == (int32_t)r) {
          const double v = vals[b + s * ELL_B];
          if (v != 0.0) out = fabs(v);
          break;
        }
    }
    d[r] = out;
  }
}

static int ell_plan_columns(mfem_context_s* ctx, mfem_csr_s* A) {
  A->ell_state = -1;
  const int K = A->max_row_nnz;
  if (A->n < 1 || K < 1 || K > 128) return MFEM_OK;
  const int64_t npad = (A->n + ELL_B - 1) & ~(int64_t)(ELL_B - 1);
  if ((double)K * (double)npad > 1.10 * (double)A->nnz + 64.0 * K) return MFEM_OK;
  MFEM_CHECK_HIP(hipMalloc(&A->ell_cols, sizeof(int32_t) * (size_t)K * (size_t)npad));
  const int grid = mfem_grid_for(npad, MFEM_BLOCK, ctx->num_cus * 16);
  mfem_by_rowptr(A, [&](auto t) {
    hipLaunchKernelGGL(k_ell_cols<decltype(t)>, dim3(grid), dim3(MFEM_BLOCK), 0, ctx->stream, A->n, npad, K, (const decltype(t)*)A->rowptr, A->colidx,
                       A->index_base, A->ell_cols);
  });
  MFEM_CHECK_LAUNCH();
  A->ell_K = K;
  A->ell_npad = npad;
  A->ell_state = 1;
  return MFEM_OK;
}
int mfem_ell_plan(mfem_context_s* ctx, mfem_csr_s* A) {
  if (A->ell_state != 0) return MFEM_OK;
  if (A->n < g_layout_min_rows_dia && A->n < g_layout_min_rows_cols) return MFEM_OK;
  struct Undo {
    mfem_csr_s* A;
    ~Undo() {
      if (!A) return;
      mfem_ell_free(A);
      A->sym_state = A->symp_state = 0;
    }
  } undo{A};
  int rc = ell_plan_columns(ctx, A);
  if (!rc && A->ell_state == 1) rc = mfem_dia_plan(ctx, A);
  if (!rc) undo.A = nullptr;
  return rc;
}

bool mfem_dia_layout_planned(const mfem_csr_s* A) { return A->ell_state == 1 && g_ell.enable && A->dia_state == 1 && g_ell.dia; }
DiaKernel mfem_dia_kernel_wanted(const mfem_csr_s* A, DiaKernel refused, bool* direct) {
  DiaKernel k = DIA_ROWS;
  if (A->dia_triples && g_ell.shared_x) {
    k = DIA_ROWS_TRIPLES;
    if (refused != DIA_SYM27 && mfem_sym_wanted(A, DIA_SYM27)) k = DIA_SYM27;
    if (refused == DIA_NONE && mfem_sym_wanted(A, DIA_SYMP)) k = DIA_SYMP;
  }
  if (direct) *direct = k == DIA_SYMP && g_ell.symp_direct;
  return k;
}
#define SYMP_BANDS2_MIN_ROWS 100000000
int mfem_symp_bands_wanted(const mfem_csr_s* A) {
  if (g_ell.symp_bands) return g_ell.symp_bands;
  return A->symp_state == 1 && (int64_t)(A->symp_p1 - A->symp_p0) * A->symp_PL >= SYMP_BANDS2_MIN_ROWS ? 2 : 1;
}
int mfem_symp_bands(const mfem_csr_s* A) { return A->symp_B ? A->symp_B : mfem_symp_bands_wanted(A); }
#define SYMP_TRIM_MIN_ROWS 16000000
int mfem_symp_trim_wanted(const mfem_csr_s* A) {
  if (g_ell.symp_trim) return g_ell.symp_trim == 1 ? 1 : 0;
  return A->symp_state == 1 && (int64_t)(A->symp_p1 - A->symp_p0) * A->symp_PL >= SYMP_TRIM_MIN_ROWS ? 1 : 0;
}
int mfem_symp_trim(const mfem_csr_s* A) { return A->symp_B ? A->symp_trim : mfem_symp_trim_wanted(A); }
static std::atomic<long long> g_symp_trim_binds{0};
extern "C" long long mfem_debug_symp_trim_count(void) { return g_symp_trim_binds; }
int mfem_symp_coded_wanted(DiaKernel k, bool fast, const double* ssym) { return k == DIA_SYMP && fast && ssym && g_ell.symp_coded ? 1 : 0; }
int mfem_symp_coded(const mfem_csr_s* A) { return A->symp_vals ? A->symp_DC : A->symp_dc_last; }
static std::atomic<long long> g_symp_coded_binds{0};
extern "C" long long mfem_debug_symp_coded_count(void) { return g_symp_coded_binds; }
static std::atomic<long long> g_symp_const_binds{0}, g_symp_const_steps{0};
extern "C" long long mfem_debug_symp_const_count(void) { return g_symp_const_binds; }
extern "C" long long mfem_debug_symp_const_steps(void) { return g_symp_const_steps; }
size_t mfem_ell_vals_bytes(const mfem_csr_s* A) {
  if (A->ell_state != 1 || !g_ell.enable) return 0;
  const bool dia = mfem_dia_layout_planned(A);
  if (A->n < (dia ? g_layout_min_rows_dia : g_layout_min_rows_cols)) return 0;
  size_t bytes = sizeof(double) * (size_t)A->ell_K * (size_t)A->ell_npad;
  if (dia && mfem_dia_kernel_wanted(A) == DIA_SYMP) {
    size_t pm = 0;
    for (int B = 1; B <= SP_BMAX; ++B)
      for (int trim = 0; trim <= 1; ++trim) pm = std::max(pm, sizeof(double) * (size_t)mfem_symp_copy_doubles(A, B, trim));
    bytes += pm;
  }
  return bytes;
}
static int dia_bind(mfem_context_s* ctx, mfem_csr_s* A, const double* vals, double* buf, const double* dsc, const double* ssym) {
  bool direct = false, fp_made = false, flags_made = false;
  SympConst cst{};
  int64_t flagged = 0;
  DiaKernel k = mfem_dia_kernel_wanted(A, DIA_NONE, &direct);
  A->symp_trim = mfem_symp_trim_wanted(A);
  A->symp_B = mfem_symp_bands_wanted(A);
  A->symp_DC = mfem_symp_coded_wanted(k, mfem_dia_fill_fast(A, dsc, direct), ssym);
  A->symp_dneg = 0;
  double* pvals = buf + (size_t)A->ell_K * (size_t)A->ell_npad;
  SympGeom G = k == DIA_SYMP ? mfem_symp_geom(ctx, A) : SympGeom{};
  auto rim_of = [&](const SympGeom& g) -> double* { return k == DIA_SYMP && g.rim_units > 0 ? pvals + (int64_t)g.NR * g.NPk * (g.p1 - g.p0) * sp_step(g.B, g.DC) : nullptr; };
  auto flags_of = [&](const SympGeom& g) -> unsigned char* { return k == DIA_SYMP && direct && g_ell.symp_const != 2 ? mfem_symp_flags_of(pvals, g) : nullptr; };
  int rc = mfem_dia_copy(ctx, A, vals, buf, dsc, ssym, G, direct ? pvals : nullptr, rim_of(G), g_ell.symp_fingerprint != 0, &fp_made, flags_of(G), &flags_made);
  while (!rc && (k == DIA_SYMP || k == DIA_SYM27)) {
    bool ok = false, dc_refused = false;
    rc = mfem_sym_verdict(ctx, A, k, buf, pvals, G, direct, fp_made, &ok, &dc_refused, &A->symp_dneg, flags_made, &cst, &flagged);
    if (rc) break;
    if (dc_refused) {
      A->symp_DC = 0;
      G = mfem_symp_geom(ctx, A);
      rc = mfem_dia_copy(ctx, A, vals, buf, dsc, ssym, G, pvals, rim_of(G), g_ell.symp_fingerprint != 0, &fp_made, flags_of(G), &flags_made);
      continue;
    }
    if (ok) break;
    if (k == DIA_SYMP && direct) rc = mfem_dia_copy(ctx, A, vals, buf, dsc, ssym, SympGeom{}, nullptr, nullptr, false, &fp_made);
    k = mfem_dia_kernel_wanted(A, k);
  }
  if (rc) return rc;
  A->ell_vals = buf;
  A->ell_src = vals;
  A->ell_bound_mode = 2;
  A->dia_kernel = k;
  A->symp_vals = k == DIA_SYMP ? pvals : nullptr;
  if (k != DIA_SYMP) A->symp_B = A->symp_DC = A->symp_trim = 0;
  if (!A->symp_DC) A->symp_dneg = 0;
  A->symp_CS = 0;
  A->symp_flagged = 0;
  if (k == DIA_SYMP) {
    const int64_t steps = mfem_symp_steps(A);
    if (!flags_made) flagged = 0;
    bool mirror = fp_made || flagged == 0;
    for (int sl = 0; sl < 13 && mirror && flagged > 0; ++sl) mirror = memcmp(&cst.v[sl], &cst.v[26 - sl], sizeof(double)) == 0;
    A->symp_CS = spc_form(flags_made && mirror, flags_made && cst.valid != 0, flagged, steps, g_ell.symp_const == 2, g_ell.symp_const == 1);
    A->symp_flagged = flagged;
    memcpy(A->symp_cst, cst.v, sizeof(A->symp_cst));
    A->symp_ccode = cst.code;
    A->symp_cs_last = A->symp_CS;
    A->symp_flagged_last = flagged;
    g_symp_const_steps = flagged;
    if (A->symp_CS) ++g_symp_const_binds;
    A->symp_dc_last = A->symp_DC;
    if (A->symp_DC) ++g_symp_coded_binds;
    if (G.rim_units > 0) ++g_symp_trim_binds;
  }
  return MFEM_OK;
}

int mfem_ell_bind(mfem_context_s* ctx, mfem_csr_s* A, const double* vals, double* buf, const double* dsc, const double* ssym) {
  mfem_ell_unbind(A);
  if (A->ell_state != 1 || !g_ell.enable || !buf) return MFEM_OK;
  if (mfem_dia_layout_planned(A)) return dia_bind(ctx, A, vals, buf, dsc, ssym);
  int waves = 4;
  while (waves > 1 && sizeof(double) * 64 * (size_t)A->ell_K * waves > 64 * 1024) waves >>= 1;
  const size_t lds = sizeof(double) * 64 * (size_t)A->ell_K * waves;
  const int64_t ntiles = A->ell_npad >> 6;
  int grid = (int)((ntiles + waves - 1) / waves);
  if (grid > ctx->num_cus * 16) grid = ctx->num_cus * 16;
  mfem_by_rowptr(A, [&](auto t) {
    hipLaunchKernelGGL(k_ell_vals_lds<decltype(t)>, dim3(grid), dim3(64 * waves), lds, ctx->stream, A->n, A->ell_npad, A->ell_K,
                       (const decltype(t)*)A->rowptr, vals, A->index_base, buf, A->colidx, dsc);
  });
  MFEM_CHECK_LAUNCH();
  A->ell_vals = buf;
  A->ell_src = vals;
  A->ell_bound_mode = 1;
  return MFEM_OK;
}
void mfem_ell_unbind(mfem_csr_s* A) {
  A->ell_bound_mode = A->dia_kernel = DIA_NONE;
  A->ell_vals = A->symp_vals = nullptr;
  A->ell_src = nullptr;
  A->symp_B = A->symp_DC = A->symp_dneg = A->symp_trim = A->symp_CS = 0;
  A->symp_flagged = 0;
}
void mfem_ell_free(mfem_csr_s* A) {
  if (A->ell_cols) hipFree(A->ell_cols);
  if (A->dia_flags) hipFree(A->dia_flags);
  if (A->dia_dev) hipFree(A->dia_dev);
  A->ell_cols = nullptr;
  A->dia_flags = nullptr;
  A->dia_dev = nullptr;
  A->ell_state = A->dia_state = 0;
}
int mfem_ell_diag(mfem_context_s* ctx, mfem_csr_s* A, double* d) {
  if (!A->ell_vals) return MFEM_ERR_INVALID;
  const int grid = mfem_grid_for(A->n, MFEM_BLOCK, ctx->num_cus * 16);
  hipLaunchKernelGGL(k_ell_diag, dim3(grid), dim3(MFEM_BLOCK), 0, ctx->stream, A->n, A->ell_K, (const DiaOffsets*)A->dia_dev,
                     A->ell_bound_mode == 2 ? A->dia_flags : nullptr, A->ell_cols, A->ell_vals, d);
  MFEM_CHECK_LAUNCH();
  return MFEM_OK;
}

static std::atomic<int64_t> g_sym_launches{0};
extern "C" int64_t mfem_debug_sym_spmv_count(void) { return g_sym_launches; }
int mfem_spmv_ell_launch(mfem_context_s* ctx, mfem_csr_s* A, const double* vals, const double* x, double* y, double alpha, double beta,
                         const double* dotw, double* partials, int* n_partials, const int32_t* done_flag, const SpmvPart& part) {
  if (!A->ell_vals || vals != A->ell_src) return 0;
  int cap = ctx->num_cus * g_ell.grid_mult;
  if (cap > MFEM_MAX_PARTIALS) cap = MFEM_MAX_PARTIALS;
  if (part.part != 0) cap /= 2;
  if (part.part == 2) {
    int64_t rows = 0;
    for (int z = 0; z < part.nz; ++z) rows += part.hi[z] - part.lo[z];
    const int64_t want = rows / 512 + 2 * part.nz + 1;
    if (want < cap) cap = (int)want;
  }
  const SpmvArgs a{x, y, alpha, beta, dotw, partials, n_partials, done_flag, part};
  int rc = MFEM_OK;
  switch (A->ell_bound_mode == 2 ? A->dia_kernel : DIA_NONE) {
    case DIA_SYMP:
    case DIA_SYM27:
      if (part.part != 2) ++g_sym_launches;
      rc = mfem_sym_launch(ctx, A, (DiaKernel)A->dia_kernel, a);
      break;
    case DIA_ROWS_TRIPLES:
    case DIA_ROWS: rc = mfem_dia_launch(ctx, A, A->dia_kernel == DIA_ROWS_TRIPLES, cap, a); break;
    default: {
      const int grid = mfem_grid_for((A->n + 1) / 2, MFEM_BLOCK, cap);
      hipLaunchKernelGGL((k_spmv_ell<2, 1>), dim3(grid), dim3(MFEM_BLOCK), 0, ctx->stream, A->n, A->ell_npad, A->ell_K, A->ell_cols, A->ell_vals, x,
                         y, alpha, beta, dotw, partials, done_flag, part);
      MFEM_CHECK_LAUNCH();
      if (n_partials && partials) *n_partials = grid;
    }
  }
  return rc ? rc : 1;
}

int64_t mfem_ell_entries(const mfem_context_s* ctx, const mfem_csr_s* A, int32_t* sweep) {
  const DiaKernel k = mfem_dia_layout_planned(A) ? mfem_dia_kernel_wanted(A) : DIA_NONE;
  if (sweep) *sweep = k == DIA_SYMP ? 2 : k == DIA_SYM27 ? 1 : 0;
  return k == DIA_SYMP || k == DIA_SYM27 ? mfem_sym_entries(ctx, A, k) : (int64_t)A->ell_K * A->ell_npad;
}
int64_t mfem_ell_design_bytes(const mfem_context_s* ctx, const mfem_csr_s* A) {
  int32_t sym = 0;
  const int64_t ent = mfem_ell_entries(ctx, A, &sym);
  if (!mfem_dia_layout_planned(A)) return ent * 12 + A->n * 16;
  const int64_t reg = (int64_t)A->dia_regular_blocks * 128;
  int64_t b = ent * 8 + A->n * 16 + (A->n > reg ? A->n - reg : 0) * (int64_t)A->ell_K * 4;
  if (sym == 2) b += mfem_symp_steps(A) * (int64_t)sp_xn(mfem_symp_bands(A)) * 8 - mfem_symp_swept_rows(A) * 8;
  return b;
}
```

metafem.jl_amd/csrc/spmv_sym.hip:

```cpp
#include "blas1.h"
#include "spmv_ell.h"

#define SYM_ROWS 512
#define SYM_THREADS (SYM_ROWS / 2)
#define SYM_WG_PER_CU 3
__global__ __launch_bounds__(SYM_THREADS) void k_spmv_sym27(int64_t n, int64_t npad, int K, const DiaOffsets* __restrict__ Op,
                                                             const int32_t* __restrict__ flags, const int32_t* __restrict__ cols,
                                                             const double* __restrict__ vals, const double* __restrict__ x,
                                                             double* __restrict__ y, double alpha, double beta,
                                                             const double* __restrict__ dotw, double* __restrict__ partials,
                                                             const int32_t* __restrict__ done_flag, int64_t c0, int64_t c1, int S, int nsteps, int cls, int gs,
                                                             int part) {
  __shared__ __attribute__((aligned(16))) double hist[9][SYM_ROWS];
  __shared__ __attribute__((aligned(16))) double exch[4][SYM_ROWS];
  __shared__ double red[16];
  if (done_flag && done_flag[0]) return;
  const int32_t* off = Op->off[cls];
  const int tid = threadIdx.x;
  double dot_acc = 0.0;
  const int tile = blockIdx.x % S, seg = blockIdx.x / S;
  const int nseg = gs / S + (tile < gs % S ? 1 : 0);
  const int seg_len = part == 2 ? 0 : (nsteps + nseg - 1) / nseg;
  bool have_hist = false;
  e_d2 up_next[4] = {{0.0, 0.0}, {0.0, 0.0}, {0.0, 0.0}, {0.0, 0.0}};
  {
    const int64_t chunk = c0 + tile + (int64_t)S * ((int64_t)seg * seg_len);
    if (part != 2 && seg * seg_len < nsteps && chunk < c1) {
      const double* v = vals + ell_base(chunk * SYM_ROWS + 2 * tid, K);
#pragma unroll
      for (int u = 0; u < 4; ++u) up_next[u] = SYM_LD(reinterpret_cast<const e_d2*>(v + (14 + u) * ELL_B));
    }
  }
  for (int it = 0; it < seg_len; ++it) {
    const int step = seg * seg_len + it;
    const int64_t chunk = c0 + tile + (int64_t)S * step;
    if (step >= nsteps || chunk >= c1) break;
    const int64_t r = chunk * SYM_ROWS + 2 * tid;
    const double* v = vals + ell_base(r, K);
    e_d2 acc = {0.0, 0.0};
    e_d2 up[4];
#pragma unroll
    for (int u = 0; u < 4; ++u) {
      up[u] = up_next[u];
      *reinterpret_cast<e_d2*>(&exch[u][2 * tid]) = up[u];
    }
    __syncthreads();
    auto slot = [&](int s, const double* tab, int lp, bool ok) -> e_d2 {
      e_d2 w;
      if (ok && lp >= 0 && lp + 1 < SYM_ROWS) {
        w.x = tab[lp];
        w.y = tab[lp + 1];
      } else {
        w = SYM_LD(reinterpret_cast<const e_d2*>(v + s * ELL_B));
      }
      return w;
    };
#define SYM_RUN(va, vb, vc, s0)                                          \
  {                                                                      \
    const u_d2* xp = reinterpret_cast<const u_d2*>(x + r + off[s0]);     \
    const u_d2 xa = xp[0], xb = xp[1];                                   \
    acc.x += va.x != 0.0 ? va.x * xa.x : 0.0;                            \
    acc.y += va.y != 0.0 ? va.y * xa.y : 0.0;                            \
    acc.x += vb.x != 0.0 ? vb.x * xa.y : 0.0;                            \
    acc.y += vb.y != 0.0 ? vb.y * xb.x : 0.0;                            \
    acc.x += vc.x != 0.0 ? vc.x * xb.x : 0.0;                            \
    acc.y += vc.y != 0.0 ? vc.y * xb.y : 0.0;                            \
    if (s0 == 12) {                                                      \
      xself0 = xa.y;                                                     \
      xself1 = xb.x;                                                     \
    }                                                                    \
  }
    double xself0 = 0.0, xself1 = 0.0;
    const int lph = 2 * tid + S * SYM_ROWS;
#pragma unroll
    for (int s = 0; s < 9; s += 3) {
      const e_d2 va = slot(s, hist[8 - s], lph + off[s], have_hist);
      const e_d2 vb = slot(s + 1, hist[7 - s], lph + off[s + 1], have_hist);
      const e_d2 vc = slot(s + 2, hist[6 - s], lph + off[s + 2], have_hist);
      SYM_RUN(va, vb, vc, s);
    }
    {
      const e_d2 va = slot(9, exch[3], 2 * tid + off[9], true);
      const e_d2 vb = slot(10, exch[2], 2 * tid + off[10], true);
      const e_d2 vc = slot(11, exch[1], 2 * tid + off[11], true);
      SYM_RUN(va, vb, vc, 9);
    }
    {
      e_d2 va;
      va.y = up[0].x;
      if (tid > 0) va.x = exch[0][2 * tid - 1];
      else va.x = v[12 * ELL_B];
      const e_d2 vb = SYM_LD(reinterpret_cast<const e_d2*>(v + 13 * ELL_B));
      SYM_RUN(va, vb, up[0], 12);
    }
    SYM_RUN(up[1], up[2], up[3], 15);
    if (it + 1 < seg_len && step + 1 < nsteps && chunk + S < c1) {
      const double* vn = vals + ell_base((chunk + S) * SYM_ROWS + 2 * tid, K);
#pragma unroll
      for (int u = 0; u < 4; ++u) up_next[u] = SYM_LD(reinterpret_cast<const e_d2*>(vn + (14 + u) * ELL_B));
    }
    __syncthreads();
#pragma unroll
    for (int s = 18; s < 27; s += 3) {
      const e_d2 va = SYM_LD(reinterpret_cast<const e_d2*>(v + s * ELL_B));
      const e_d2 vb = SYM_LD(reinterpret_cast<const e_d2*>(v + (s + 1) * ELL_B));
      const e_d2 vc = SYM_LD(reinterpret_cast<const e_d2*>(v + (s + 2) * ELL_B));
      SYM_RUN(va, vb, vc, s);
      *reinterpret_cast<e_d2*>(&hist[s - 18][2 * tid]) = va;
      *reinterpret_cast<e_d2*>(&hist[s - 17][2 * tid]) = vb;
      *reinterpret_cast<e_d2*>(&hist[s - 16][2 * tid]) = vc;
    }
#undef SYM_RUN
    have_hist = true;
    double y0 = alpha * acc.x, y1 = alpha * acc.y;
    if (beta != 0.0) {
      y0 += beta * y[r];
      y1 += beta * y[r + 1];
    }
    y[r] = y0;
    y[r + 1] = y1;
    if (dotw) {
      if (dotw == x) dot_acc += y0 * xself0 + y1 * xself1;
      else dot_acc += y0 * dotw[r] + y1 * dotw[r + 1];
    }
  }
  if (part != 1) {
    const int64_t nchunks = (n + SYM_ROWS - 1) / SYM_ROWS;
    for (int64_t q = blockIdx.x;; q += gridDim.x) {
      const int64_t ch = q < c0 ? q : c1 + (q - c0);
      if (ch >= nchunks) break;
      const int64_t r = ch * SYM_ROWS + 2 * tid;
      if (r < n) dia_rows<2, 3, true>(r, n, npad, K, *Op, flags, cols, vals, x, y, alpha, beta, dotw, 0, dot_acc);
    }
  }
  if (partials) {
    const double b = block_reduce_sum(dot_acc, red);
    if (threadIdx.x == 0) partials[blockIdx.x] = b;
  }
}

__global__ __launch_bounds__(MFEM_BLOCK) void k_sym27_check(int K, const DiaOffsets* __restrict__ Op, const double* __restrict__ vals,
                                                              int64_t row_lo, int64_t row_hi, int cls, int32_t* __restrict__ bad) {
  const int32_t* off = Op->off[cls];
  const int64_t stride = (int64_t)gridDim.x * blockDim.x;
  int fail = 0;
  for (int64_t r = row_lo + blockIdx.x * (int64_t)blockDim.x + threadIdx.x; r < row_hi; r += stride) {
    const double* v = vals + ell_base(r, K);
    for (int s = 0; s < 13; ++s) {
      const int64_t rs = r + off[s];
      if (rs < row_lo) continue;
      const double a = v[s * ELL_B], b = vals[ell_base(rs, K) + (26 - s) * ELL_B];
      if (__double_as_longlong(a) != __double_as_longlong(b) && !(a == 0.0 && b == 0.0)) fail = 1;
    }
  }
  if (fail) atomicOr(bad, 1);
}


__constant__ int32_t c_sp_ecell[SP_BMAX][sp_epad(SP_BMAX)];
static int symp_upload_tables(int device) {
  static bool done[64] = {};
  if (device >= 0 && device < 64 && done[device]) return MFEM_OK;
  int32_t h[SP_BMAX][sp_epad(SP_BMAX)];
  for (int B = 1; B <= SP_BMAX; ++B)
    for (int e = 0; e < sp_epad(SP_BMAX); ++e) {
      int s_, l_, c_, cell = 0;
      h[B - 1][e] = sp_edge(e, s_, l_, c_, cell, B) ? cell : sp_tab(B);
    }
  MFEM_CHECK_HIP(hipMemcpyToSymbol(HIP_SYMBOL(c_sp_ecell), h, sizeof(h)));
  if (device >= 0 && device < 64) done[device] = true;
  return MFEM_OK;
}

__device__ __forceinline__ void symp_rim_unit(const SympGeom& Gm, const double* __restrict__ rimv, int64_t u, int lane, const double* __restrict__ x,
                                              double* __restrict__ y, double alpha, double beta, const double* __restrict__ dotw, double& dot_acc) {
  const int64_t g = u * SPT_UNIT + lane;
  if (g >= Gm.rim_rows) return;
  const int pl = (int)(g / Gm.rim_pp);
  int j = 0, k = 0;
  spt_rim_row((int)(g - (int64_t)pl * Gm.rim_pp), Gm.m2, Gm.ms1, Gm.ms2, j, k);
  const int64_t r = (int64_t)(Gm.p0 + pl) * Gm.PL + (int64_t)j * Gm.m2 + k;
  const double* v = rimv + u * SPT_UNIT_DOUBLES + lane;
  double vv[27], xv[27];
#pragma unroll
  for (int s = 0; s < 27; ++s) {
    vv[s] = SYM_LD(v + s * SPT_UNIT);
    int64_t idx = r + (int64_t)(s / 9 - 1) * Gm.PL + (int64_t)(sp_dj(s) * Gm.m2 + sp_dk(s));
    idx = idx < 0 ? 0 : idx;
    xv[s] = x[idx < Gm.nx ? idx : Gm.nx - 1];
  }
  double acc = 0.0;
#pragma unroll
  for (int s = 0; s < 27; ++s) acc += vv[s] != 0.0 ? vv[s] * xv[s] : 0.0;
  double y0 = alpha * acc;
  if (beta != 0.0) y0 += beta * y[r];
  y[r] = y0;
  if (dotw) dot_acc += y0 * dotw[r];
}
__global__ __launch_bounds__(64) void k_symp_rim(SympGeom Gm, const double* __restrict__ rimv, const double* __restrict__ x, double* __restrict__ y,
                                                  double alpha, double beta, const double* __restrict__ dotw, double* __restrict__ partials,
                                                  const int32_t* __restrict__ done_flag) {
  if (done_flag && done_flag[0]) return;
  double dot_acc = 0.0;
  for (int64_t u = blockIdx.x; u < Gm.rim_units; u += gridDim.x) symp_rim_unit(Gm, rimv, u, threadIdx.x, x, y, alpha, beta, dotw, dot_acc);
  if (partials) {
    const double w = wave_reduce_sum(dot_acc);
    if (threadIdx.x == 0) partials[blockIdx.x] = w;
  }
}

template <int MODE, int B, int DC, int CS>
__device__ __forceinline__ void symp_sweep(const SympGeom& Gm, const double* __restrict__ pv, const double* __restrict__ x,
                                           double* __restrict__ y, double alpha, double beta,
                                           const double* __restrict__ dotw, double* __restrict__ partials,
                                           const int32_t* __restrict__ done_flag, int32_t* __restrict__ bad, const SympTail& tail, const SympConst& cst,
                                           const uint32_t* __restrict__ sflags) {
  static_assert(CS == 0 || MODE == 0, "the check pass reads the stored copy");
  constexpr int XL = sp_xl(B), XN = sp_xn(B), XU = sp_xu(B), NE = sp_ne(B), EU = sp_eu(B), MAINB = sp_main(B, DC), LOWB = sp_low(B);
  constexpr int NSL = sp_nslots(DC), S0 = 27 - NSL;
  constexpr int BM = NSL * SP_ROWS, BL = 13 * SP_ROWS, BT = SP_L * SP_LS;
  __shared__ __attribute__((aligned(16))) double xs[3][XL][SP_XW];
  __shared__ __attribute__((aligned(16))) double tab[sp_tab(B) + 2 + (CS ? 28 : 0)];
  double* const ctab = tab + sp_tab(B) + 2;
  if (done_flag && done_flag[0]) return;
  const int lane = threadIdx.x, lj = lane / SP_PW, pk = lane % SP_PW, lb0 = lj * SP_LS + 2 * pk;
  const int NP = Gm.NR * Gm.NPk, nplanes = Gm.p1 - Gm.p0;
  const int xcd = blockIdx.x & 7, pc = NP / 8, prem = NP % 8, pcnt = pc + (xcd < prem ? 1 : 0), pfirst = xcd * pc + (xcd < prem ? xcd : prem);
  int ecell[EU];
#pragma unroll
  for (int u = 0; u < EU; ++u) ecell[u] = c_sp_ecell[B - 1][lane + 64 * u];
  if (CS && lane == 0) {
#pragma unroll
    for (int s = 0; s < 27; ++s) ctab[s] = cst.v[s];
  }
  int fw = 0;
  int64_t ft0 = 0;
  int cur_patch = -1, bp = 0, bc = 1, bn = 2;
  int nb = 1;
  bool have_hist = false;
  bool vxb[B], vyb[B];
  int64_t rin = 0;
  int xo[XU], xa[XU];
  double dot_acc = 0.0;
  int fail = 0;
  e_d2 cur[B][NSL];
  int cdc[B];
  e_d2 keep[3];
  double ed[EU], xr[XU];
  auto xidx = [&](int plane, int u) -> int64_t {
    int64_t idx = (int64_t)plane * Gm.PL + xo[u];
    idx = idx < 0 ? 0 : idx;
    return idx < Gm.nx ? idx : Gm.nx - 1;
  };
  auto request = [&](const double* v, int b, bool fl) {
    if (CS && fl) return;
    if (vxb[b]) {
#pragma unroll
      for (int u = 0; u < NSL; ++u) cur[b][u] = SYM_LD(reinterpret_cast<const e_d2*>(v + b * BM + 2 * lane + u * SP_ROWS));
      if (DC && MODE == 0) cdc[b] = SYM_LD(reinterpret_cast<const unsigned short*>(v + sp_coff(B, DC)) + b * (SP_ROWS / 2) + lane);
    } else {
#pragma unroll
      for (int u = 0; u < NSL; ++u) cur[b][u] = (e_d2){0.0, 0.0};
      if (DC) cdc[b] = 0;
    }
  };
  auto request_step = [&](const double* v, int pnext, bool fl) {
    if (MODE == 0) {
      if (!(CS && fl)) {
#pragma unroll
        for (int u = 0; u < EU - 1; ++u) ed[u] = SYM_LD(v + B * BM + lane + 64 * u);
        ed[EU - 1] = lane < NE - 64 * (EU - 1) ? SYM_LD(v + B * BM + lane + 64 * (EU - 1)) : 0.0;
      }
#pragma unroll
      for (int u = 0; u < XU - 1; ++u) xr[u] = x[xidx(pnext, u)];
      xr[XU - 1] = lane < XN - 64 * (XU - 1) ? x[xidx(pnext, XU - 1)] : 0.0;
    }
  };
  auto stage_x = [&](int buf, int plane) {
    double* dst = &xs[buf][0][0];
#pragma unroll
    for (int u = 0; u < XU - 1; ++u) dst[xa[u]] = x[xidx(plane, u)];
    if (lane < XN - 64 * (XU - 1)) dst[xa[XU - 1]] = x[xidx(plane, XU - 1)];
  };
  const int W = gridDim.x >> 3, jw = blockIdx.x >> 3, rot = spc_rot(Gm.NPk);
  for (int rk = 0; W * rk < pcnt * Gm.nseg; ++rk) {
  const int run = spc_run(W, jw, rk, rot);
  if (run >= pcnt * Gm.nseg) continue;
  const int patch = pfirst + run % pcnt, seg = run / pcnt;
  const int64_t t0 = (int64_t)patch * nplanes + (int64_t)nplanes * seg / Gm.nseg, t1 = (int64_t)patch * nplanes + (int64_t)nplanes * (seg + 1) / Gm.nseg;
  cur_patch = -1;
  for (int64_t t = t0; t < t1; ++t) {
    const int p = Gm.p0 + (int)(t - (int64_t)patch * nplanes);
    const int64_t step = (int64_t)(p - Gm.p0) * NP + patch;
    const double* v = pv + step * MAINB;
    const double* vlow = pv + (int64_t)NP * nplanes * MAINB + step * LOWB;
    const bool more = t + 1 < t1 && p + 1 < Gm.p1;
    if (CS && (patch != cur_patch || t - ft0 >= 63)) {
      ft0 = t;
      const int64_t tl = t + lane, sl = (tl - (int64_t)patch * nplanes) * NP + patch;
      fw = tl < t1 ? (int)((sflags[sl >> 2] >> (8 * (int)(sl & 3))) & 255u) : 0;
    }
    const bool fnow = CS && __builtin_amdgcn_readlane(fw, (int)(t - ft0)) != 0;
    const bool fnext = CS && more && __builtin_amdgcn_readlane(fw, (int)(t + 1 - ft0)) != 0;
    if (patch != cur_patch) {
      cur_patch = patch;
      const int j0 = (patch / Gm.NPk) * (SP_L * B), k0 = (patch % Gm.NPk) * SP_W;
      const int k = k0 + 2 * pk;
      nb = 1;
#pragma unroll
      for (int b = 0; b < B; ++b) {
        const int j = j0 + SP_L * b + lj;
        vxb[b] = j < Gm.m1 && k < Gm.m2;
        vyb[b] = j < Gm.m1 && k + 1 < Gm.m2;
        if (b > 0 && j0 + SP_L * b < Gm.m1) nb = b + 1;
      }
      rin = (int64_t)(j0 + lj) * Gm.m2 + k;
#pragma unroll
      for (int u = 0; u < XU; ++u) {
        const int tt = lane + 64 * u, xl = tt / SP_XC, xc = tt - SP_XC * xl;
        xo[u] = (j0 - 1 + xl) * Gm.m2 + (k0 - 1 + xc);
        xa[u] = xl * SP_XW + xc;
      }
      have_hist = false;
      __syncthreads();
#pragma unroll
      for (int b = 0; b < B; ++b)
        if (b < nb) request(v, b, fnow);
      request_step(v, p + 1, fnow);
      if (MODE == 0) {
        stage_x(bp, p - 1);
        stage_x(bc, p);
#pragma unroll
        for (int b = 0; b < B; ++b) {
          if (b < nb && !fnow) {
#pragma unroll
            for (int s = 0; s < 9; ++s) {
              const e_d2 w = vxb[b] ? SYM_LD(reinterpret_cast<const e_d2*>(vlow + b * BL + 2 * lane + s * SP_ROWS)) : (e_d2){0.0, 0.0};
              double* c = tab + sp_tbase(s, B) + (sp_dj(s) + sp_adj(s)) * SP_LS + sp_dk(s) + 2 + b * BT + lb0;
              c[0] = w.x;
              c[1] = w.y;
            }
          }
        }
      }
    }
    if (CS && fnow) {
      {
        double* dst = &xs[bn][0][0];
#pragma unroll
        for (int u = 0; u < XU - 1; ++u) dst[xa[u]] = xr[u];
        if (lane < XN - 64 * (XU - 1)) dst[xa[XU - 1]] = xr[XU - 1];
      }
      __syncthreads();
      if (more && fnext) request_step(v + (int64_t)NP * MAINB, p + 2, true);
#pragma unroll
      for (int b = 0; b < B; ++b) {
        e_d2 acc = {0.0, 0.0};
        double xself0 = 0.0, xself1 = 0.0;
        auto crun = [&](int s, int buf, int dj, bool self) {
#pragma clang fp contract(off)
          const double* xp = &xs[buf][SP_L * b + lj + 1 + dj][2 * pk];
          const e_d2 xa2 = *reinterpret_cast<const e_d2*>(xp), xb2 = *reinterpret_cast<const e_d2*>(xp + 2);
          const double c0 = ctab[s], c1 = ctab[s + 1], c2 = ctab[s + 2];
          acc.x = acc.x + c0 * xa2.x;
          acc.y = acc.y + c0 * xa2.y;
          acc.x = acc.x + c1 * xa2.y;
          acc.y = acc.y + c1 * xb2.x;
          acc.x = acc.x + c2 * xb2.x;
          acc.y = acc.y + c2 * xb2.y;
          if (self) {
            xself0 = xa2.y;
            xself1 = xb2.x;
          }
        };
        crun(0, bp, -1, false);
        crun(3, bp, 0, false);
        crun(6, bp, 1, false);
        crun(9, bc, -1, false);
        crun(12, bc, 0, true);
        crun(15, bc, 1, false);
        crun(18, bn, -1, false);
        crun(21, bn, 0, false);
        crun(24, bn, 1, false);
        const int64_t r = (int64_t)p * Gm.PL + rin + (int64_t)(SP_L * b) * Gm.m2;
        double y0 = alpha * acc.x, y1 = alpha * acc.y;
        if (beta != 0.0) {
          y0 += beta * y[r];
          y1 += beta * y[r + 1];
        }
        __builtin_nontemporal_store((u_d2){y0, y1}, reinterpret_cast<u_d2*>(y + r));
        if (dotw) {
          if (dotw == x) {
            dot_acc += y0 * xself0;
            dot_acc += y1 * xself1;
          } else {
            dot_acc += y0 * dotw[r];
            dot_acc += y1 * dotw[r + 1];
          }
        }
      }
      __syncthreads();
      const int b_ = bp;
      bp = bc;
      bc = bn;
      bn = b_;
      if (!(more && fnext)) cur_patch = -1;
      continue;
    }
#pragma unroll
    for (int b = 0; b < B; ++b) {
    if (b < nb) {
    const int lb = lb0 + b * BT;
    const bool vx = vxb[b], vy = vyb[b], lastb = b + 1 >= nb;
#pragma unroll
    for (int s = 9; s < 13; ++s) *reinterpret_cast<e_d2*>(tab + sp_tbase(s, B) + sp_adj(s) * SP_LS + 2 + lb) = cur[b][26 - s - S0];
    e_d2 low[13];
    if (MODE == 0) {
      if (b == 0) {
#pragma unroll
        for (int u = 0; u < EU; ++u) tab[ecell[u]] = ed[u];
        double* dst = &xs[bn][0][0];
#pragma unroll
        for (int u = 0; u < XU - 1; ++u) dst[xa[u]] = xr[u];
        if (lane < XN - 64 * (XU - 1)) dst[xa[XU - 1]] = xr[XU - 1];
      }
    } else {
#pragma unroll
      for (int s = 0; s < 13; ++s) low[s] = vx ? SYM_LD(reinterpret_cast<const e_d2*>(vlow + b * BL + 2 * lane + s * SP_ROWS)) : (e_d2){0.0, 0.0};
    }
    e_d2 mine[NSL];
#pragma unroll
    for (int u = 0; u < NSL; ++u) mine[u] = cur[b][u];
    const int mcd = DC && MODE == 0 ? cdc[b] : 0;
    __syncthreads();
    if (more) {
      request(v + (int64_t)NP * MAINB, b, fnext);
      if (lastb) request_step(v + (int64_t)NP * MAINB, p + 2, fnext);
    }
    auto mirrored = [&](int s) -> e_d2 {
      const double* c = tab + sp_tbase(s, B) + (sp_dj(s) + sp_adj(s)) * SP_LS + sp_dk(s) + 2 + lb;
      e_d2 w;
      w.x = c[0];
      w.y = c[1];
      return w;
    };
    e_d2 acc = {0.0, 0.0};
    double xself0 = 0.0, xself1 = 0.0;
    auto run = [&](const e_d2& va, const e_d2& vb, const e_d2& vc, int buf, int dj, bool self) {
#pragma clang fp contract(off)
      const double* xp = &xs[buf][SP_L * b + lj + 1 + dj][2 * pk];
      const e_d2 xa2 = *reinterpret_cast<const e_d2*>(xp), xb2 = *reinterpret_cast<const e_d2*>(xp + 2);
      acc.x = acc.x + va.x * xa2.x;
      acc.y = acc.y + va.y * xa2.y;
      acc.x = acc.x + vb.x * xa2.y;
      acc.y = acc.y + vb.y * xb2.x;
      acc.x = acc.x + vc.x * xb2.x;
      acc.y = acc.y + vc.y * xb2.y;
      if (self) {
        xself0 = xa2.y;
        xself1 = xb2.x;
      }
    };
    if (MODE == 1) {
#pragma unroll
      for (int s = 0; s < 13; ++s) {
        const int dj = sp_dj(s), dk = sp_dk(s), gl = SP_L * b + lj;
        const bool in = gl + dj >= 0 && gl + dj < SP_L * nb && (dk < 0 ? pk > 0 : dk > 0 ? pk < SP_PW - 1 : true);
        if (in && vx && (s >= 9 || have_hist)) {
          const e_d2 m = mirrored(s);
          if (__double_as_longlong(m.x) != __double_as_longlong(low[s].x) && !(m.x == 0.0 && low[s].x == 0.0)) fail = 1;
          if (vy && __double_as_longlong(m.y) != __double_as_longlong(low[s].y) && !(m.y == 0.0 && low[s].y == 0.0)) fail = 1;
        }
      }
    } else {
      run(mirrored(0), mirrored(1), mirrored(2), bp, -1, false);
      run(mirrored(3), mirrored(4), mirrored(5), bp, 0, false);
      run(mirrored(6), mirrored(7), mirrored(8), bp, 1, false);
      run(mirrored(9), mirrored(10), mirrored(11), bc, -1, false);
      e_d2 dg;
      if (DC) {
        dg.x = __longlong_as_double(Gm.unit + (long long)(signed char)(mcd & 255));
        dg.y = __longlong_as_double(Gm.unit + (long long)(signed char)((mcd >> 8) & 255));
      } else {
        dg = mine[0];
      }
      run(mirrored(12), dg, mine[14 - S0], bc, 0, true);
      run(mine[15 - S0], mine[16 - S0], mine[17 - S0], bc, 1, false);
    }
    __syncthreads();
#pragma unroll
    for (int s = 3; s < 9; ++s) *reinterpret_cast<e_d2*>(tab + sp_tbase(s, B) + sp_adj(s) * SP_LS + 2 + lb) = mine[26 - s - S0];
    if (B > 1 && !lastb) {
#pragma unroll
      for (int s = 0; s < 3; ++s) keep[s] = mine[26 - s - S0];
    } else {
#pragma unroll
      for (int s = 0; s < 3; ++s) {
        *reinterpret_cast<e_d2*>(tab + sp_tbase(s, B) + sp_adj(s) * SP_LS + 2 + lb) = mine[26 - s - S0];
        if (B > 1 && b > 0) *reinterpret_cast<e_d2*>(tab + sp_tbase(s, B) + sp_adj(s) * SP_LS + 2 + lb - BT) = keep[s];
      }
    }
    if (MODE == 0) {
      run(mine[18 - S0], mine[19 - S0], mine[20 - S0], bn, -1, false);
      run(mine[21 - S0], mine[22 - S0], mine[23 - S0], bn, 0, false);
      run(mine[24 - S0], mine[25 - S0], mine[26 - S0], bn, 1, false);
      const int64_t r = (int64_t)p * Gm.PL + rin + (int64_t)(SP_L * b) * Gm.m2;
      double y0 = alpha * acc.x, y1 = alpha * acc.y;
      if (beta != 0.0) {
        if (vx) y0 += beta * y[r];
        if (vy) y1 += beta * y[r + 1];
      }
      {
        if (vy) __builtin_nontemporal_store((u_d2){y0, y1}, reinterpret_cast<u_d2*>(y + r));
        else if (vx) __builtin_nontemporal_store(y0, y + r);
      }
      if (dotw) {
        if (dotw == x) {
          if (vx) dot_acc += y0 * xself0;
          if (vy) dot_acc += y1 * xself1;
        } else {
          if (vx) dot_acc += y0 * dotw[r];
          if (vy) dot_acc += y1 * dotw[r + 1];
        }
      }
    }
    }
    }
    have_hist = true;
    if (MODE == 0) {
      const int b_ = bp;
      bp = bc;
      bc = bn;
      bn = b_;
    }
    if (!more) cur_patch = -1;
  }
  }
  if (MODE == 0 && tail.on) {
    const int64_t UA = (tail.lo + 127) / 128, ub = tail.hi / 128, UB = (tail.n + 127) / 128 - ub;
    for (int64_t u = blockIdx.x; u < UA + UB; u += gridDim.x) {
      const int64_t r = (u < UA ? u : ub + (u - UA)) * 128 + 2 * lane;
      if (r < tail.n)
        dia_rows<2, 3, true>(r, tail.n, tail.npad, tail.K, *tail.Op, tail.flags, tail.cols, tail.ell, x, y, alpha, beta, dotw, 0, dot_acc,
                             tail.lo, tail.hi);
    }
  }
  if (MODE == 0 && tail.rim) {
    const double* rimv = pv + (int64_t)NP * nplanes * (MAINB + LOWB);
    for (int64_t u = blockIdx.x; u < Gm.rim_units; u += gridDim.x) symp_rim_unit(Gm, rimv, u, lane, x, y, alpha, beta, dotw, dot_acc);
  }
  if (MODE == 1) {
    if (fail) atomicOr(bad, 1);
  } else if (partials) {
    const double w = wave_reduce_sum(dot_acc);
    if (lane == 0) partials[blockIdx.x] = w;
  }
}

template <int MODE, int B, int DC>
__global__ __launch_bounds__(64) void k_spmv_symp(SympGeom Gm, const double* __restrict__ pv, const double* __restrict__ x,
                                                   double* __restrict__ y, double alpha, double beta,
                                                   const double* __restrict__ dotw, double* __restrict__ partials,
                                                   const int32_t* __restrict__ done_flag, int32_t* __restrict__ bad, SympTail tail) {
  symp_sweep<MODE, B, DC, 0>(Gm, pv, x, y, alpha, beta, dotw, partials, done_flag, bad, tail, SympConst{}, nullptr);
}
template <int B, int DC>
__global__ __launch_bounds__(64) void k_spmv_symp_const(SympGeom Gm, const double* __restrict__ pv, const double* __restrict__ x,
                                                         double* __restrict__ y, double alpha, double beta,
                                                         const double* __restrict__ dotw, double* __restrict__ partials,
                                                         const int32_t* __restrict__ done_flag, SympTail tail, SympConst cst,
                                                         const uint32_t* __restrict__ sflags) {
  symp_sweep<0, B, DC, 1>(Gm, pv, x, y, alpha, beta, dotw, partials, done_flag, nullptr, tail, cst, sflags);
}

__global__ __launch_bounds__(MFEM_BLOCK) void k_symp_bind(SympGeom Gm, int K, const double* __restrict__ ell, double* __restrict__ pv) {
  const int lane = threadIdx.x & 63, lj = lane / SP_PW, pk = lane % SP_PW;
  const int NP = Gm.NR * Gm.NPk, B = Gm.B;
  const int MAINB = sp_main(B), LOWB = sp_low(B), NEB = sp_ne(B), EPADB = sp_epad(B);
  const int64_t T = (int64_t)NP * (Gm.p1 - Gm.p0);
  for (int64_t t = (int64_t)blockIdx.x * (MFEM_BLOCK / 64) + (threadIdx.x >> 6); t < T; t += (int64_t)gridDim.x * (MFEM_BLOCK / 64)) {
    const int nplanes = Gm.p1 - Gm.p0, patch = (int)(t / nplanes), p = Gm.p0 + (int)(t % nplanes);
    const int j0 = (patch / Gm.NPk) * (SP_L * B), k0 = (patch % Gm.NPk) * SP_W;
    const int64_t step = (int64_t)(p - Gm.p0) * NP + patch;
    double* out = pv + step * MAINB;
    double* outlow = pv + T * MAINB + step * LOWB;
    for (int b = 0; b < B; ++b) {
      const int j = j0 + SP_L * b + lj, k = k0 + 2 * pk;
      const bool vx = j < Gm.m1 && k < Gm.m2, vy = j < Gm.m1 && k + 1 < Gm.m2;
      const int64_t r = (int64_t)p * Gm.PL + (int64_t)j * Gm.m2 + k;
      const int64_t b0 = ell_base(r, K), b1 = ell_base(r + 1, K);
      for (int s0 = 0; s0 < 27; s0 += 9) {
        e_d2 w[9];
#pragma unroll
        for (int u = 0; u < 9; ++u) {
          w[u].x = vx ? ell[b0 + (s0 + u) * ELL_B] : 0.0;
          w[u].y = vy ? ell[b1 + (s0 + u) * ELL_B] : 0.0;
        }
#pragma unroll
        for (int u = 0; u < 9; ++u) {
          const int sl = s0 + u;
          double* dst = sl < 13 ? outlow + b * 13 * SP_ROWS + sl * SP_ROWS : out + b * 14 * SP_ROWS + (sl - 13) * SP_ROWS;
          *reinterpret_cast<e_d2*>(dst + 2 * lane) = w[u];
        }
      }
    }
    for (int e = lane; e < EPADB; e += 64) {
      int s = 0, line = 0, col = 0, cell = 0;
      double val = 0.0;
      if (e < NEB && sp_edge(e, s, line, col, cell, B) && j0 + line < Gm.m1 && k0 + col < Gm.m2)
        val = ell[ell_base((int64_t)p * Gm.PL + (int64_t)(j0 + line) * Gm.m2 + k0 + col, K) + s * ELL_B];
      out[B * 14 * SP_ROWS + e] = val;
    }
  }
}

static void sym27_plan(mfem_csr_s* A, const int32_t* off, int lc, int64_t PL, int64_t run_lo, int64_t run_hi) {
  const int64_t Sc = (PL + SYM_ROWS / 2) / SYM_ROWS;
  if (Sc < 8 || Sc > MFEM_MAX_PARTIALS / 2) return;
  const int64_t bpc = SYM_ROWS / ELL_B, c0 = (run_lo + bpc - 1) / bpc, c1 = run_hi / bpc;
  if (c1 - c0 < 4 * Sc) return;
  int64_t mx = 0, myz = 0;
  for (int t = 0; t < SYM_ROWS / 2; ++t) {
    for (int q = 0; q < 9; ++q) {
      const int64_t lp = 2 * t + Sc * SYM_ROWS + off[q];
      if (lp >= 0 && lp + 1 < SYM_ROWS) mx += 2;
    }
    for (int q = 9; q < 12; ++q) {
      const int64_t lp = 2 * t + off[q];
      if (lp >= 0 && lp + 1 < SYM_ROWS) myz += 2;
    }
    myz += t > 0 ? 2 : 1;
  }
  if (20 * (mx + myz) < 5 * 13 * SYM_ROWS) return;
  A->sym_state = 1;
  A->sym_c0 = c0;
  A->sym_c1 = c1;
  A->sym_S = (int)Sc;
  A->sym_cls = lc;
  A->sym_mx = mx;
  A->sym_myz = myz;
}
static void symp_plan(mfem_csr_s* A, int lc, int64_t m2, int64_t PL, int64_t run_lo, int64_t run_hi) {
  A->symp_state = -1;
  if (PL % m2 != 0 || PL / m2 < 2 || PL >= (int64_t)1 << 30) return;
  const int64_t p0 = (run_lo * ELL_B + PL - 1) / PL, p1 = run_hi * ELL_B / PL;
  if (p1 - p0 < 4 || p0 < 1) return;
  A->symp_state = 1;
  A->symp_m2 = (int)m2;
  A->symp_m1 = (int)(PL / m2);
  A->symp_PL = PL;
  A->symp_p0 = (int)p0;
  A->symp_p1 = (int)p1;
  A->symp_NS = (A->symp_m1 + SP_L - 1) / SP_L;
  A->symp_NPk = (A->symp_m2 + SP_W - 1) / SP_W;
  A->sym_cls = lc;
}
void mfem_sym_plan(mfem_csr_s* A, const int32_t* off, int lc, int64_t m2, int64_t PL, int64_t run_lo, int64_t run_hi) {
  sym27_plan(A, off, lc, PL, run_lo, run_hi);
  symp_plan(A, lc, m2, PL, run_lo, run_hi);
}

bool mfem_sym_wanted(const mfem_csr_s* A, DiaKernel k) {
  if (!g_ell.sym || !A->dia_triples) return false;
  const bool all = g_layout_min_rows_dia == 0;
  if (k == DIA_SYM27) return A->sym_state == 1 && (all || A->sym_c1 - A->sym_c0 >= 2700);
  return A->symp_state == 1 && g_ell.symp && (all || (int64_t)(A->symp_p1 - A->symp_p0) * A->symp_PL >= 24000000 || A->symp_m2 > 256);
}

static int sym27_grid(const mfem_context_s* ctx, const mfem_csr_s* A, int64_t* nsteps_out) {
  const int64_t nsteps = (A->sym_c1 - A->sym_c0 + A->sym_S - 1) / A->sym_S;
  const int resident = SYM_WG_PER_CU * ctx->num_cus;
  int nseg = resident / A->sym_S;
  if (nseg < 1) nseg = 1;
  if ((int64_t)A->sym_S * nseg * 10 < (int64_t)resident * 8) nseg = (8 * ctx->num_cus + A->sym_S - 1) / A->sym_S;
  while (nseg > 1 && (int64_t)A->sym_S * nseg > MFEM_MAX_PARTIALS - 512) --nseg;
  if (nseg > nsteps / 8) nseg = (int)(nsteps / 8);
  if (nseg < 1) nseg = 1;
  if (nsteps_out) *nsteps_out = nsteps;
  return A->sym_S * nseg;
}
struct SympExt { int ms1, ms2, NS, NPk, NR; };
static SympExt symp_ext(const mfem_csr_s* A, int B, int trim) {
  SympExt e;
  e.ms1 = spt_ms1(A->symp_m1, B, trim != 0);
  e.ms2 = spt_ms2(A->symp_m2, trim != 0);
  e.NS = (e.ms1 + SP_L - 1) / SP_L;
  e.NPk = spt_cols(e.ms2);
  e.NR = spt_rows(e.ms1, B);
  return e;
}
static SympExt symp_ext(const mfem_csr_s* A) { return symp_ext(A, mfem_symp_bands(A), mfem_symp_trim(A)); }
static int symp_nseg(const mfem_context_s* ctx, const mfem_csr_s* A) {
  const SympExt e = symp_ext(A);
  return spt_nseg((int64_t)e.NR * e.NPk, (int64_t)sp_wg_per_cu(mfem_symp_bands(A)) * ctx->num_cus, A->symp_p1 - A->symp_p0);
}
SympGeom mfem_symp_geom(const mfem_context_s* ctx, const mfem_csr_s* A) {
  const int B = mfem_symp_bands(A);
  const SympExt e = symp_ext(A);
  SympGeom G{A->symp_PL, A->n, A->symp_m1, A->symp_m2, A->symp_p0, A->symp_p1, e.NS, e.NPk, symp_nseg(ctx, A), B, e.NR, A->symp_DC, sp_unit_bits(A->symp_dneg)};
  G.ms1 = e.ms1;
  G.ms2 = e.ms2;
  G.rim_pp = spt_rim(G.m1, G.m2, G.ms1, G.ms2);
  G.rim_rows = (int64_t)G.rim_pp * (G.p1 - G.p0);
  G.rim_units = spt_units(G.rim_rows);
  return G;
}
int64_t mfem_symp_steps(const mfem_csr_s* A, int B, int trim) {
  if (B < 1) B = mfem_symp_bands(A);
  const SympExt e = symp_ext(A, B, trim < 0 ? mfem_symp_trim(A) : trim);
  return (int64_t)e.NR * e.NPk * (A->symp_p1 - A->symp_p0);
}
int64_t mfem_symp_copy_doubles(const mfem_csr_s* A, int B, int trim) {
  const SympExt e = symp_ext(A, B, trim);
  return mfem_symp_steps(A, B, trim) * sp_step(B) + spt_units((int64_t)spt_rim(A->symp_m1, A->symp_m2, e.ms1, e.ms2) * (A->symp_p1 - A->symp_p0)) * SPT_UNIT_DOUBLES +
         spc_flag_doubles(mfem_symp_steps(A, B, trim));
}
unsigned char* mfem_symp_flags_of(double* pvals, const SympGeom& G) {
  return (unsigned char*)(pvals + (int64_t)G.NR * G.NPk * (G.p1 - G.p0) * sp_step(G.B, G.DC) + G.rim_units * SPT_UNIT_DOUBLES);
}
int64_t mfem_symp_swept_rows(const mfem_csr_s* A) {
  const SympExt e = symp_ext(A);
  return (int64_t)(A->symp_p1 - A->symp_p0) * e.ms1 * e.ms2;
}
#define SYMP_RIM_GRID 256
static int symp_grid(const mfem_context_s* ctx, const mfem_csr_s* A) {
  const int B = mfem_symp_bands(A);
  const SympExt e = symp_ext(A);
  const int64_t NP = (int64_t)e.NR * e.NPk;
  int64_t g = 8 * ((NP + 7) / 8) * symp_nseg(ctx, A);
  int64_t cap = (int64_t)sp_wg_per_cu(B) * ctx->num_cus;
  if (cap > MFEM_MAX_PARTIALS - 1024 - SYMP_RIM_GRID) cap = MFEM_MAX_PARTIALS - 1024 - SYMP_RIM_GRID;
  cap &= ~(int64_t)7;
  if (g > cap) g = cap;
  return g < 8 ? 8 : (int)g;
}

int64_t mfem_sym_entries(const mfem_context_s* ctx, const mfem_csr_s* A, DiaKernel k) {
  if (k == DIA_SYM27) {
    const int64_t nch = A->sym_c1 - A->sym_c0;
    return (int64_t)A->ell_K * A->ell_npad - ((nch - sym27_grid(ctx, A, nullptr)) * A->sym_mx + nch * A->sym_myz);
  }
  const int B = mfem_symp_bands(A);
  const SympExt x = symp_ext(A);
  const int NP = x.NR * x.NPk, nplanes = A->symp_p1 - A->symp_p0, nseg = symp_nseg(ctx, A);
  int64_t e = (int64_t)A->ell_K * (A->ell_npad - (int64_t)nplanes * A->symp_PL), codes = 0;
  e += 27 * (int64_t)spt_rim(A->symp_m1, A->symp_m2, x.ms1, x.ms2) * nplanes;
  for (int patch = 0; patch < NP; ++patch) {
    int64_t nv = 0;
    for (int lp = 0; lp < 64 * B; ++lp) {
      const int j = (patch / x.NPk) * (SP_L * B) + lp / SP_PW, kk = (patch % x.NPk) * SP_W + 2 * (lp % SP_PW);
      if (j < A->symp_m1 && kk < A->symp_m2) ++nv;
    }
    e += (28 * nv + sp_ne(B)) * nplanes + 18 * nv * nseg;
    codes += 2 * nv * nplanes;
  }
  if (A->symp_vals ? A->symp_CS : A->symp_cs_last) {
    const int64_t fl = A->symp_vals ? A->symp_flagged : A->symp_flagged_last;
    e -= fl * spc_saved_entries(B) - spc_flag_doubles((int64_t)NP * nplanes);
    codes -= fl * spc_saved_codes(B);
  }
  if (mfem_symp_coded(A)) e -= codes - (codes + 7) / 8;
  return e;
}

static auto symp_const_kernel(const SympGeom& G) {
  if (G.DC) return G.B == 2 ? k_spmv_symp_const<2, 1> : k_spmv_symp_const<1, 1>;
  return G.B == 2 ? k_spmv_symp_const<2, 0> : k_spmv_symp_const<1, 0>;
}
template <int MODE>
static auto symp_kernel(const SympGeom& G) {
  if (G.DC) return G.B == 2 ? k_spmv_symp<MODE, 2, 1> : k_spmv_symp<MODE, 1, 1>;
  return G.B == 2 ? k_spmv_symp<MODE, 2, 0> : k_spmv_symp<MODE, 1, 0>;
}

static std::atomic<long long> g_symp_fp_checks{0};
extern "C" long long mfem_debug_symp_fingerprint_count(void) { return g_symp_fp_checks; }

int mfem_sym_verdict(mfem_context_s* ctx, mfem_csr_s* A, DiaKernel k, const double* buf, double* pvals, const SympGeom& G, bool direct, bool fp_made, bool* ok,
                     bool* dc_refused, int* dneg, bool flags_made, SympConst* cst, int64_t* flagged) {
  int32_t* d_bad = ctx->d_flags + 9;
  const size_t fp_ints = flags_made && k == DIA_SYMP ? MFEM_NFLAGS - 16 : 4;
  auto read_const = [&]() {
    if (!(flags_made && k == DIA_SYMP && cst && flagged)) return;
    *flagged = ctx->h_flags[SPC_COUNT_AT];
    memcpy(cst, ctx->h_flags + SPC_REF_AT, sizeof(SympConst));
  };
  *dc_refused = false;
  *dneg = 0;
  if (k == DIA_SYMP) {
    { const int rt = symp_upload_tables(ctx->device); if (rt) return rt; }
    if (!direct) {
      const int64_t T = mfem_symp_steps(A);
      const int gb = (int)(T / 4 + 1 < (int64_t)ctx->num_cus * 32 ? T / 4 + 1 : (int64_t)ctx->num_cus * 32);
      hipLaunchKernelGGL(k_symp_bind, dim3(gb), dim3(MFEM_BLOCK), 0, ctx->stream, G, A->ell_K, buf, pvals);
      MFEM_CHECK_LAUNCH();
    }
    if (fp_made) {
      MFEM_CHECK_HIP(hipMemcpyAsync(ctx->h_flags + 16, ctx->d_flags + 16, fp_ints * sizeof(int32_t), hipMemcpyDeviceToHost, ctx->stream));
      MFEM_CHECK_HIP(hipStreamSynchronize(ctx->stream));
      unsigned long long fpv;
      memcpy(&fpv, ctx->h_flags + 16, sizeof(fpv));
      *ok = fpv == 0;
      *dc_refused = G.DC && ctx->h_flags[18] != 0;
      *dneg = G.DC && ctx->h_flags[19] != 0;
      read_const();
      ++g_symp_fp_checks;
      return MFEM_OK;
    }
  }
  MFEM_CHECK_HIP(hipMemsetAsync(d_bad, 0, sizeof(int32_t), ctx->stream));
  if (k == DIA_SYMP)
    hipLaunchKernelGGL(symp_kernel<1>(G), dim3(symp_grid(ctx, A)), dim3(64), 0, ctx->stream, G, (const double*)pvals,
                       (const double*)nullptr, (double*)nullptr, 0.0, 0.0, (const double*)nullptr, (double*)nullptr, (const int32_t*)nullptr, d_bad,
                       SympTail{});
  else
    hipLaunchKernelGGL(k_sym27_check, dim3(ctx->num_cus * 8), dim3(MFEM_BLOCK), 0, ctx->stream, A->ell_K, (const DiaOffsets*)A->dia_dev, buf,
                       A->sym_c0 * SYM_ROWS, A->sym_c1 * SYM_ROWS, A->sym_cls, d_bad);
  MFEM_CHECK_LAUNCH();
  MFEM_CHECK_HIP(hipMemcpyAsync(ctx->h_flags + 9, d_bad, sizeof(int32_t), hipMemcpyDeviceToHost, ctx->stream));
  if (k == DIA_SYMP && (G.DC || flags_made)) MFEM_CHECK_HIP(hipMemcpyAsync(ctx->h_flags + 18, ctx->d_flags + 18, (fp_ints - 2) * sizeof(int32_t), hipMemcpyDeviceToHost, ctx->stream));
  MFEM_CHECK_HIP(hipStreamSynchronize(ctx->stream));
  *ok = ctx->h_flags[9] == 0;
  *dc_refused = k == DIA_SYMP && G.DC && ctx->h_flags[18] != 0;
  *dneg = k == DIA_SYMP && G.DC && ctx->h_flags[19] != 0;
  read_const();
  return MFEM_OK;
}

int mfem_sym_launch(mfem_context_s* ctx, mfem_csr_s* A, DiaKernel k, const SpmvArgs& a) {
  const DiaOffsets* O = (const DiaOffsets*)A->dia_dev;
  int np = 0;
  if (k == DIA_SYM27) {
    int64_t nsteps = 0;
    const int gs = sym27_grid(ctx, A, &nsteps);
    const int64_t outside = (A->n + SYM_ROWS - 1) / SYM_ROWS - (A->sym_c1 - A->sym_c0);
    np = a.part.part == 2 ? (int)(outside < 1 ? 1 : outside < 512 ? outside : 512) : gs;
    hipLaunchKernelGGL(k_spmv_sym27, dim3(np), dim3(SYM_THREADS), 0, ctx->stream, A->n, A->ell_npad, A->ell_K, O, A->dia_flags, A->ell_cols, A->ell_vals,
                       a.x, a.y, a.alpha, a.beta, a.dotw, a.partials, a.done_flag, A->sym_c0, A->sym_c1, A->sym_S, (int)nsteps, A->sym_cls, gs, a.part.part);
    MFEM_CHECK_LAUNCH();
  } else {
    const SympGeom G = mfem_symp_geom(ctx, A);
    const int64_t lo = (int64_t)G.p0 * G.PL, hi = (int64_t)G.p1 * G.PL;
    SympTail tl{};
    if (a.part.part == 0 && g_ell.symp_tail) tl = SympTail{1, A->ell_K, G.rim_units > 0, A->n, A->ell_npad, lo, hi, O, A->dia_flags, A->ell_cols, A->ell_vals};
    if (a.part.part != 2) {
      np = symp_grid(ctx, A);
      if (A->symp_CS) {
        SympConst cst{};
        memcpy(cst.v, A->symp_cst, sizeof(cst.v));
        cst.code = A->symp_ccode;
        cst.valid = 1;
        hipLaunchKernelGGL(symp_const_kernel(G), dim3(np), dim3(64), 0, ctx->stream, G, (const double*)A->symp_vals, a.x, a.y, a.alpha, a.beta, a.dotw,
                           a.partials, a.done_flag, tl, cst, (const uint32_t*)mfem_symp_flags_of(A->symp_vals, G));
      } else {
        hipLaunchKernelGGL(symp_kernel<0>(G), dim3(np), dim3(64), 0, ctx->stream, G, (const double*)A->symp_vals, a.x, a.y, a.alpha, a.beta, a.dotw,
                           a.partials, a.done_flag, (int32_t*)nullptr, tl);
      }
      MFEM_CHECK_LAUNCH();
    }
    if (a.part.part == 2 || (a.part.part == 0 && !tl.on)) {
      int go = 0;
      const int rc = mfem_dia_launch_outside(ctx, A, a, a.partials ? a.partials + np : nullptr, lo, hi, &go);
      if (rc) return rc;
      np += go;
      if (G.rim_units > 0) {
        const int gr = (int)(G.rim_units < SYMP_RIM_GRID ? G.rim_units : SYMP_RIM_GRID);
        hipLaunchKernelGGL(k_symp_rim, dim3(gr), dim3(64), 0, ctx->stream, G, (const double*)A->symp_vals + (int64_t)G.NR * G.NPk * (G.p1 - G.p0) * sp_step(G.B, G.DC),
                           a.x, a.y, a.alpha, a.beta, a.dotw, a.partials ? a.partials + np : nullptr, a.done_flag);
        MFEM_CHECK_LAUNCH();
        np += gr;
      }
    }
  }
  if (a.n_partials && a.partials) *a.n_partials = np;
  return MFEM_OK;
}
```

Before: 34.51 billion DOF-updates/s.

## Add cost-balanced static schedule of symp runs across waves

Measured after the change: 37.41 billion DOF-updates/s, median of 6. 8.4% higher.

```diff
diff --git a/include/metafem_mi355x_debug.h b/include/metafem_mi355x_debug.h
--- a/include/metafem_mi355x_debug.h
+++ b/include/metafem_mi355x_debug.h
@@ -17,6 +17,7 @@
                                   const double* dotw, double* partials_out , int32_t cap, int32_t* n_partials , int32_t* form );
 int mfem_debug_set(const char* key, int64_t a, int64_t b);
 
+long long mfem_debug_symp_sched_count(void);
 int mfem_debug_lat27_cg_fused(void);
 int64_t mfem_debug_lat27_pass1_bytes(mfem_csr A);
 long long mfem_debug_lat27_spmv_count(void);
diff --git a/metafem.jl_amd/_lib.py b/metafem.jl_amd/_lib.py
--- a/metafem.jl_amd/_lib.py
+++ b/metafem.jl_amd/_lib.py
@@ -174,6 +174,7 @@
     "mfem_debug_symp_trim_count": (C.c_longlong, []),
     "mfem_debug_symp_const_count": (C.c_longlong, []),
     "mfem_debug_symp_const_steps": (C.c_longlong, []),
+    "mfem_debug_symp_sched_count": (C.c_longlong, []),
     "mfem_debug_spmv_scaled_layout": (c_int, [P, P, P, P, P, P, c_double, c_double, P, P, c_int32, C.POINTER(c_int32), C.POINTER(c_int32)]),
     "mfem_debug_set": (c_int, [C.c_char_p, c_int64, c_int64]),
     "mfem_debug_graph_comm_count": (c_int, []),
diff --git a/metafem.jl_amd/csrc/api.hip b/metafem.jl_amd/csrc/api.hip
--- a/metafem.jl_amd/csrc/api.hip
+++ b/metafem.jl_amd/csrc/api.hip
@@ -305,6 +305,7 @@
 extern "C" {
 int mfem_debug_set_spmv(int, int);
 int mfem_debug_set_ell(int);
+int mfem_debug_set_symp_sched(int64_t, int64_t);
 int mfem_debug_set_sell(int);
 int mfem_debug_set_lat27(int);
 int mfem_debug_set_lat8(int);
@@ -336,6 +337,7 @@
   const std::string k(key);
   if (k == "spmv") return mfem_debug_set_spmv((int)a, (int)b);
   if (k == "ell") return mfem_debug_set_ell((int)a);
+  if (k == "symp_sched") return mfem_debug_set_symp_sched(a, b);
   if (k == "sell") return mfem_debug_set_sell((int)a);
   if (k == "lat27") return mfem_debug_set_lat27((int)a);
   if (k == "lat8") return mfem_debug_set_lat8((int)a);
diff --git a/metafem.jl_amd/csrc/common.h b/metafem.jl_amd/csrc/common.h
--- a/metafem.jl_amd/csrc/common.h
+++ b/metafem.jl_amd/csrc/common.h
@@ -174,6 +174,8 @@
   int64_t symp_flagged, symp_flagged_last;
   double symp_cst[27];
   int symp_ccode;
+  const int32_t* symp_sched;
+  int symp_sched_grid;
   int symp_dc_last;
   double* symp_vals;
   SellLayout sell;
diff --git a/metafem.jl_amd/csrc/krylov.h b/metafem.jl_amd/csrc/krylov.h
--- a/metafem.jl_amd/csrc/krylov.h
+++ b/metafem.jl_amd/csrc/krylov.h
@@ -82,6 +82,7 @@
   key = mfem_hash(key, A->symp_B + 16 * A->symp_DC + 32 * A->symp_dneg + 64 * A->symp_trim);
   key = mfem_hash(key, A->symp_CS);
   if (A->symp_CS) { key = mfem_hash_bytes(key, A->symp_cst, sizeof(A->symp_cst)); key = mfem_hash(key, A->symp_ccode); }
+  key = mfem_hash(key, A->symp_sched); key = mfem_hash(key, A->symp_sched_grid);
   key = mfem_hash(key, A->lat27.dsc); key = mfem_hash(key, A->lat8.dsc);
   key = mfem_hash(key, A->rem_active);
   key = mfem_hash(key, A->op != nullptr); key = mfem_hash(key, A->op_epoch); key = mfem_hash(key, A->op_scratch); key = mfem_hash(key, A->op_dsc);
diff --git a/metafem.jl_amd/csrc/spmv_ell.h b/metafem.jl_amd/csrc/spmv_ell.h
--- a/metafem.jl_amd/csrc/spmv_ell.h
+++ b/metafem.jl_amd/csrc/spmv_ell.h
@@ -5,6 +5,7 @@
 #include "spmv_symp.h"
 #include "symp_trim_decide.h"
 #include "symp_const_decide.h"
+#include "symp_sched_decide.h"
 
 #define ELL_B 128
 __host__ __device__ __forceinline__ int64_t ell_base(int64_t r, int K) { return (r >> 7) * ((int64_t)K * ELL_B) + (r & (ELL_B - 1)); }
@@ -206,4 +207,5 @@
 int mfem_sym_verdict(mfem_context_s* ctx, mfem_csr_s* A, DiaKernel k, const double* buf, double* pvals, const SympGeom& G, bool direct, bool fp_made, bool* ok,
                      bool* dc_refused, int* dneg, bool flags_made = false, SympConst* cst = nullptr, int64_t* flagged = nullptr);
 unsigned char* mfem_symp_flags_of(double* pvals, const SympGeom& G);
+int mfem_symp_sched_bind(mfem_context_s* ctx, mfem_csr_s* A, const SympGeom& G);
 int mfem_sym_launch(mfem_context_s* ctx, mfem_csr_s* A, DiaKernel k, const SpmvArgs& a);
diff --git a/metafem.jl_amd/csrc/spmv_ell.hip b/metafem.jl_amd/csrc/spmv_ell.hip
--- a/metafem.jl_amd/csrc/spmv_ell.hip
+++ b/metafem.jl_amd/csrc/spmv_ell.hip
@@ -331,6 +331,7 @@
     A->symp_dc_last = A->symp_DC;
     if (A->symp_DC) ++g_symp_coded_binds;
     if (G.rim_units > 0) ++g_symp_trim_binds;
+    return mfem_symp_sched_bind(ctx, A, G);
   }
   return MFEM_OK;
 }
@@ -361,6 +362,8 @@
   A->ell_src = nullptr;
   A->symp_B = A->symp_DC = A->symp_dneg = A->symp_trim = A->symp_CS = 0;
   A->symp_flagged = 0;
+  A->symp_sched = nullptr;
+  A->symp_sched_grid = 0;
 }
 void mfem_ell_free(mfem_csr_s* A) {
   if (A->ell_cols) hipFree(A->ell_cols);
diff --git a/metafem.jl_amd/csrc/spmv_sym.hip b/metafem.jl_amd/csrc/spmv_sym.hip
--- a/metafem.jl_amd/csrc/spmv_sym.hip
+++ b/metafem.jl_amd/csrc/spmv_sym.hip
@@ -209,13 +209,23 @@
   }
 }
 
-template <int MODE, int B, int DC, int CS>
+#ifdef SYMP_SCHED_CLOCKS
+__device__ long long* g_symp_clocks = nullptr;
+__device__ int g_symp_clocks_runs = 0;
+extern "C" int mfem_debug_symp_clocks(long long* buf , int runs) {
+  if (!buf || runs < 0) runs = 0;
+  if (hipMemcpyToSymbol(HIP_SYMBOL(g_symp_clocks_runs), &runs, sizeof(runs)) != hipSuccess) return MFEM_ERR_HIP;
+  return hipMemcpyToSymbol(HIP_SYMBOL(g_symp_clocks), &buf, sizeof(buf)) == hipSuccess ? MFEM_OK : MFEM_ERR_HIP;
+}
+#endif
+template <int MODE, int B, int DC, int CS, int SCH>
 __device__ __forceinline__ void symp_sweep(const SympGeom& Gm, const double* __restrict__ pv, const double* __restrict__ x,
                                            double* __restrict__ y, double alpha, double beta,
                                            const double* __restrict__ dotw, double* __restrict__ partials,
                                            const int32_t* __restrict__ done_flag, int32_t* __restrict__ bad, const SympTail& tail, const SympConst& cst,
-                                           const uint32_t* __restrict__ sflags) {
+                                           const uint32_t* __restrict__ sflags, const int32_t* __restrict__ sched, int nruns_pr) {
   static_assert(CS == 0 || MODE == 0, "the check pass reads the stored copy");
+  static_assert(SCH == 0 || CS == 1, "only the constant form is scheduled");
   constexpr int XL = sp_xl(B), XN = sp_xn(B), XU = sp_xu(B), NE = sp_ne(B), EU = sp_eu(B), MAINB = sp_main(B, DC), LOWB = sp_low(B);
   constexpr int NSL = sp_nslots(DC), S0 = 27 - NSL;
   constexpr int BM = NSL * SP_ROWS, BL = 13 * SP_ROWS, BT = SP_L * SP_LS;
@@ -283,10 +293,28 @@
     if (lane < XN - 64 * (XU - 1)) dst[xa[XU - 1]] = x[xidx(plane, XU - 1)];
   };
   const int W = gridDim.x >> 3, jw = blockIdx.x >> 3, rot = spc_rot(Gm.NPk);
-  for (int rk = 0; W * rk < pcnt * Gm.nseg; ++rk) {
-  const int run = spc_run(W, jw, rk, rot);
-  if (run >= pcnt * Gm.nseg) continue;
-  const int patch = pfirst + run % pcnt, seg = run / pcnt;
+  int l0 = 0, nlist = (pcnt * Gm.nseg + W - 1) / W, lw = 0;
+  if (SCH) {
+    const int ov = lane < 2 ? sched[blockIdx.x + lane] : 0;
+    l0 = __builtin_amdgcn_readlane(ov, 0);
+    nlist = __builtin_amdgcn_readlane(ov, 1) - l0;
+  }
+  for (int rk = 0; rk < nlist; ++rk) {
+  int patch, seg;
+  if (SCH) {
+    if ((rk & 63) == 0) lw = rk + lane < nlist ? sched[gridDim.x + 1 + l0 + rk + lane] : 0;
+    const int rid = __builtin_amdgcn_readlane(lw, rk & 63);
+    patch = rid / Gm.nseg;
+    seg = rid - patch * Gm.nseg;
+  } else {
+    const int run = spc_run(W, jw, rk, rot);
+    if (run >= pcnt * Gm.nseg) continue;
+    patch = pfirst + run % pcnt;
+    seg = run / pcnt;
+  }
+#ifdef SYMP_SCHED_CLOCKS
+  const long long clk0 = wall_clock64();
+#endif
   const int64_t t0 = (int64_t)patch * nplanes + (int64_t)nplanes * seg / Gm.nseg, t1 = (int64_t)patch * nplanes + (int64_t)nplanes * (seg + 1) / Gm.nseg;
   cur_patch = -1;
   for (int64_t t = t0; t < t1; ++t) {
@@ -535,6 +563,20 @@
     }
     if (!more) cur_patch = -1;
   }
+  if (MODE == 0 && nruns_pr > 0 && partials) {
+    const double w = wave_reduce_sum(dot_acc);
+    if (lane == 0) partials[sps_run_id(patch, seg, Gm.nseg)] = w;
+    dot_acc = 0.0;
+  }
+#ifdef SYMP_SCHED_CLOCKS
+  if (MODE == 0 && nruns_pr > 0 && g_symp_clocks && sps_run_id(patch, seg, Gm.nseg) < g_symp_clocks_runs && lane == 0) {
+    long long* c = g_symp_clocks + 4 * (int64_t)sps_run_id(patch, seg, Gm.nseg);
+    c[0] = clk0;
+    c[1] = wall_clock64();
+    c[2] = blockIdx.x;
+    c[3] = rk;
+  }
+#endif
   }
   if (MODE == 0 && tail.on) {
     const int64_t UA = (tail.lo + 127) / 128, ub = tail.hi / 128, UB = (tail.n + 127) / 128 - ub;
@@ -553,7 +595,7 @@
     if (fail) atomicOr(bad, 1);
   } else if (partials) {
     const double w = wave_reduce_sum(dot_acc);
-    if (lane == 0) partials[blockIdx.x] = w;
+    if (lane == 0) partials[nruns_pr + blockIdx.x] = w;
   }
 }
 
@@ -561,16 +603,16 @@
 __global__ __launch_bounds__(64) void k_spmv_symp(SympGeom Gm, const double* __restrict__ pv, const double* __restrict__ x,
                                                    double* __restrict__ y, double alpha, double beta,
                                                    const double* __restrict__ dotw, double* __restrict__ partials,
-                                                   const int32_t* __restrict__ done_flag, int32_t* __restrict__ bad, SympTail tail) {
-  symp_sweep<MODE, B, DC, 0>(Gm, pv, x, y, alpha, beta, dotw, partials, done_flag, bad, tail, SympConst{}, nullptr);
-}
-template <int B, int DC>
+                                                   const int32_t* __restrict__ done_flag, int32_t* __restrict__ bad, SympTail tail, int nruns_pr) {
+  symp_sweep<MODE, B, DC, 0, 0>(Gm, pv, x, y, alpha, beta, dotw, partials, done_flag, bad, tail, SympConst{}, nullptr, nullptr, nruns_pr);
+}
+template <int B, int DC, int SCH>
 __global__ __launch_bounds__(64) void k_spmv_symp_const(SympGeom Gm, const double* __restrict__ pv, const double* __restrict__ x,
                                                          double* __restrict__ y, double alpha, double beta,
                                                          const double* __restrict__ dotw, double* __restrict__ partials,
                                                          const int32_t* __restrict__ done_flag, SympTail tail, SympConst cst,
-                                                         const uint32_t* __restrict__ sflags) {
-  symp_sweep<0, B, DC, 1>(Gm, pv, x, y, alpha, beta, dotw, partials, done_flag, nullptr, tail, cst, sflags);
+                                                         const uint32_t* __restrict__ sflags, const int32_t* __restrict__ sched, int nruns_pr) {
+  symp_sweep<0, B, DC, 1, SCH>(Gm, pv, x, y, alpha, beta, dotw, partials, done_flag, nullptr, tail, cst, sflags, sched, nruns_pr);
 }
 
 __global__ __launch_bounds__(MFEM_BLOCK) void k_symp_bind(SympGeom Gm, int K, const double* __restrict__ ell, double* __restrict__ pv) {
@@ -713,16 +755,31 @@
 int64_t mfem_symp_copy_doubles(const mfem_csr_s* A, int B, int trim) {
   const SympExt e = symp_ext(A, B, trim);
   return mfem_symp_steps(A, B, trim) * sp_step(B) + spt_units((int64_t)spt_rim(A->symp_m1, A->symp_m2, e.ms1, e.ms2) * (A->symp_p1 - A->symp_p0)) * SPT_UNIT_DOUBLES +
-         spc_flag_doubles(mfem_symp_steps(A, B, trim));
+         spc_flag_doubles(mfem_symp_steps(A, B, trim)) + SPS_TABLE_DOUBLES;
 }
 unsigned char* mfem_symp_flags_of(double* pvals, const SympGeom& G) {
   return (unsigned char*)(pvals + (int64_t)G.NR * G.NPk * (G.p1 - G.p0) * sp_step(G.B, G.DC) + G.rim_units * SPT_UNIT_DOUBLES);
+}
+static int32_t* symp_sched_of(double* pvals, const SympGeom& G) {
+  return (int32_t*)(mfem_symp_flags_of(pvals, G) + 8 * spc_flag_doubles((int64_t)G.NR * G.NPk * (G.p1 - G.p0)));
 }
 int64_t mfem_symp_swept_rows(const mfem_csr_s* A) {
   const SympExt e = symp_ext(A);
   return (int64_t)(A->symp_p1 - A->symp_p0) * e.ms1 * e.ms2;
 }
 #define SYMP_RIM_GRID 256
+static_assert(SPS_MAX_PARTIALS == MFEM_MAX_PARTIALS && SPS_OUTSIDE_RESERVE == 1024 + SYMP_RIM_GRID, "symp_sched_decide.h spells both out");
+static std::atomic<int> g_symp_sched_mode{SPS_AUTO}, g_symp_sched_cap{0};
+static std::atomic<long long> g_symp_sched_seed{0};
+extern "C" int mfem_debug_set_symp_sched(int64_t a, int64_t b) {
+  ++mfem_debug_epoch;
+  g_symp_sched_mode = (int)(a & 255);
+  g_symp_sched_seed = (long long)(a >> 8);
+  g_symp_sched_cap = b > 0 ? (int)(b < MFEM_MAX_PARTIALS ? b : MFEM_MAX_PARTIALS) : 0;
+  return MFEM_OK;
+}
+static std::atomic<long long> g_symp_sched_binds{0};
+extern "C" long long mfem_debug_symp_sched_count(void) { return g_symp_sched_binds; }
 static int symp_grid(const mfem_context_s* ctx, const mfem_csr_s* A) {
   const int B = mfem_symp_bands(A);
   const SympExt e = symp_ext(A);
@@ -730,9 +787,39 @@
   int64_t g = 8 * ((NP + 7) / 8) * symp_nseg(ctx, A);
   int64_t cap = (int64_t)sp_wg_per_cu(B) * ctx->num_cus;
   if (cap > MFEM_MAX_PARTIALS - 1024 - SYMP_RIM_GRID) cap = MFEM_MAX_PARTIALS - 1024 - SYMP_RIM_GRID;
+  if (g_symp_sched_cap > 0 && cap > g_symp_sched_cap) cap = g_symp_sched_cap;
   cap &= ~(int64_t)7;
   if (g > cap) g = cap;
   return g < 8 ? 8 : (int)g;
+}
+
+int mfem_symp_sched_bind(mfem_context_s* ctx, mfem_csr_s* A, const SympGeom& G) {
+  A->symp_sched = nullptr;
+  A->symp_sched_grid = 0;
+  if (!A->symp_vals) return MFEM_OK;
+  const SpsGeom g{G.NR * G.NPk, G.NPk, G.nseg, G.p1 - G.p0, symp_grid(ctx, A)};
+  const int kind = sps_kind(A->symp_CS != 0, sps_per_run(sps_nruns(g), g.grid, g_ell.symp_tail ? 0 : SPS_OUTSIDE_RESERVE), g_symp_sched_mode);
+  if (!kind) return MFEM_OK;
+  const int64_t steps = (int64_t)g.NP * g.nplanes;
+  const int nruns = sps_nruns(g);
+  std::vector<unsigned char> fl((size_t)steps);
+  MFEM_CHECK_HIP(hipMemcpyAsync(fl.data(), mfem_symp_flags_of(A->symp_vals, G), (size_t)steps, hipMemcpyDeviceToHost, ctx->stream));
+  MFEM_CHECK_HIP(hipStreamSynchronize(ctx->stream));
+  std::vector<int32_t> flagged((size_t)nruns), table((size_t)g.grid + 1 + nruns), work(2 * (size_t)nruns + g.grid);
+  std::vector<int64_t> load((size_t)g.grid);
+  int32_t first[9];
+  for (int p = 0; p < g.NP; ++p)
+    for (int s = 0; s < g.nseg; ++s) flagged[sps_run_id(p, s, g.nseg)] = sps_run_flagged(g, fl.data(), p, s);
+  sps_build(g, flagged.data(), kind == SPS_RANDOM ? SPS_RANDOM : SPS_AUTO, (uint64_t)g_symp_sched_seed.load(), table.data(), table.data() + g.grid + 1, first,
+            load.data(), work.data());
+  static_assert(sizeof(int32_t) * (2 * SPS_MAX_PARTIALS + 1) <= sizeof(double) * SPS_TABLE_DOUBLES, "the table's room in the layout's buffer");
+  int32_t* d = symp_sched_of(A->symp_vals, G);
+  MFEM_CHECK_HIP(hipMemcpyAsync(d, table.data(), sizeof(int32_t) * table.size(), hipMemcpyHostToDevice, ctx->stream));
+  MFEM_CHECK_HIP(hipStreamSynchronize(ctx->stream));
+  A->symp_sched = d;
+  A->symp_sched_grid = g.grid;
+  ++g_symp_sched_binds;
+  return MFEM_OK;
 }
 
 int64_t mfem_sym_entries(const mfem_context_s* ctx, const mfem_csr_s* A, DiaKernel k) {
@@ -763,9 +850,10 @@
   return e;
 }
 
+template <int SCH>
 static auto symp_const_kernel(const SympGeom& G) {
-  if (G.DC) return G.B == 2 ? k_spmv_symp_const<2, 1> : k_spmv_symp_const<1, 1>;
-  return G.B == 2 ? k_spmv_symp_const<2, 0> : k_spmv_symp_const<1, 0>;
+  if (G.DC) return G.B == 2 ? k_spmv_symp_const<2, 1, SCH> : k_spmv_symp_const<1, 1, SCH>;
+  return G.B == 2 ? k_spmv_symp_const<2, 0, SCH> : k_spmv_symp_const<1, 0, SCH>;
 }
 template <int MODE>
 static auto symp_kernel(const SympGeom& G) {
@@ -812,7 +900,7 @@
   if (k == DIA_SYMP)
     hipLaunchKernelGGL(symp_kernel<1>(G), dim3(symp_grid(ctx, A)), dim3(64), 0, ctx->stream, G, (const double*)pvals,
                        (const double*)nullptr, (double*)nullptr, 0.0, 0.0, (const double*)nullptr, (double*)nullptr, (const int32_t*)nullptr, d_bad,
-                       SympTail{});
+                       SympTail{}, 0);
   else
     hipLaunchKernelGGL(k_sym27_check, dim3(ctx->num_cus * 8), dim3(MFEM_BLOCK), 0, ctx->stream, A->ell_K, (const DiaOffsets*)A->dia_dev, buf,
                        A->sym_c0 * SYM_ROWS, A->sym_c1 * SYM_ROWS, A->sym_cls, d_bad);
@@ -844,17 +932,20 @@
     SympTail tl{};
     if (a.part.part == 0 && g_ell.symp_tail) tl = SympTail{1, A->ell_K, G.rim_units > 0, A->n, A->ell_npad, lo, hi, O, A->dia_flags, A->ell_cols, A->ell_vals};
     if (a.part.part != 2) {
-      np = symp_grid(ctx, A);
+      const int grid = symp_grid(ctx, A), nruns = G.NR * G.NPk * G.nseg;
+      const int nruns_pr = sps_per_run(nruns, grid, tl.on ? 0 : SPS_OUTSIDE_RESERVE) ? nruns : 0;
+      const int32_t* sched = nruns_pr && A->symp_CS && A->symp_sched && A->symp_sched_grid == grid ? A->symp_sched : nullptr;
+      np = nruns_pr + grid;
       if (A->symp_CS) {
         SympConst cst{};
         memcpy(cst.v, A->symp_cst, sizeof(cst.v));
         cst.code = A->symp_ccode;
         cst.valid = 1;
-        hipLaunchKernelGGL(symp_const_kernel(G), dim3(np), dim3(64), 0, ctx->stream, G, (const double*)A->symp_vals, a.x, a.y, a.alpha, a.beta, a.dotw,
-                           a.partials, a.done_flag, tl, cst, (const uint32_t*)mfem_symp_flags_of(A->symp_vals, G));
+        hipLaunchKernelGGL(sched ? symp_const_kernel<1>(G) : symp_const_kernel<0>(G), dim3(grid), dim3(64), 0, ctx->stream, G, (const double*)A->symp_vals, a.x, a.y, a.alpha, a.beta, a.dotw,
+                           a.partials, a.done_flag, tl, cst, (const uint32_t*)mfem_symp_flags_of(A->symp_vals, G), sched, nruns_pr);
       } else {
-        hipLaunchKernelGGL(symp_kernel<0>(G), dim3(np), dim3(64), 0, ctx->stream, G, (const double*)A->symp_vals, a.x, a.y, a.alpha, a.beta, a.dotw,
-                           a.partials, a.done_flag, (int32_t*)nullptr, tl);
+        hipLaunchKernelGGL(symp_kernel<0>(G), dim3(grid), dim3(64), 0, ctx->stream, G, (const double*)A->symp_vals, a.x, a.y, a.alpha, a.beta, a.dotw,
+                           a.partials, a.done_flag, (int32_t*)nullptr, tl, nruns_pr);
       }
       MFEM_CHECK_LAUNCH();
     }
diff --git a/metafem.jl_amd/csrc/symp_sched_decide.h b/metafem.jl_amd/csrc/symp_sched_decide.h
--- /dev/null
+++ b/metafem.jl_amd/csrc/symp_sched_decide.h
@@ -0,0 +1,151 @@
+#pragma once
+#include <stdint.h>
+
+#include "symp_const_decide.h"
+
+#define SPS_CU_PS 4900000
+#define SPS_CF_PS 2400000
+#define SPS_CS0_PS 0
+__host__ __device__ constexpr int64_t sps_run_cost(int64_t unflagged, int64_t flagged) { return unflagged * SPS_CU_PS + flagged * SPS_CF_PS + SPS_CS0_PS; }
+
+__host__ __device__ constexpr int sps_run_id(int patch, int seg, int nseg) { return patch * nseg + seg; }
+__host__ __device__ constexpr int sps_plane_lo(int nplanes, int seg, int nseg) { return (int)((int64_t)nplanes * seg / nseg); }
+
+#define SPS_MAX_PARTIALS 4096
+#define SPS_OUTSIDE_RESERVE 1280
+__host__ __device__ constexpr bool sps_per_run(int64_t nruns, int64_t grid, int64_t reserve) { return nruns > 0 && nruns + grid + reserve <= SPS_MAX_PARTIALS; }
+__host__ __device__ constexpr int sps_partials(int64_t nruns, int64_t grid, int64_t reserve) { return (int)(sps_per_run(nruns, grid, reserve) ? nruns + grid : grid); }
+#define SPS_TABLE_DOUBLES ((2 * SPS_MAX_PARTIALS + 2) / 2)
+
+enum { SPS_AUTO = 0, SPS_IDENTITY = 1, SPS_RANDOM = 2 };
+__host__ __device__ constexpr int sps_kind(bool constant_form, bool per_run, int mode) {
+  return !constant_form || !per_run || mode == SPS_IDENTITY ? 0 : mode == SPS_RANDOM ? SPS_RANDOM : 1;
+}
+
+__host__ __device__ constexpr int sps_eq_first(int NP, int c) { return c * (NP / 8) + (c < NP % 8 ? c : NP % 8); }
+__host__ __device__ inline bool sps_identity_run(int NP, int NPk, int nseg, int W, int xcd, int jw, int rk, int& patch, int& seg) {
+  const int first = sps_eq_first(NP, xcd), pcnt = sps_eq_first(NP, xcd + 1) - first;
+  const int run = spc_run(W, jw, rk, spc_rot(NPk));
+  if (run >= pcnt * nseg) return false;
+  patch = first + run % pcnt;
+  seg = run / pcnt;
+  return true;
+}
+__host__ __device__ constexpr int sps_identity_rounds(int NP, int nseg, int W, int xcd) {
+  return ((sps_eq_first(NP, xcd + 1) - sps_eq_first(NP, xcd)) * nseg + W - 1) / W;
+}
+
+struct SpsGeom {
+  int NP, NPk;
+  int nseg;
+  int nplanes;
+  int grid;
+};
+__host__ __device__ constexpr int sps_nruns(const SpsGeom& g) { return g.NP * g.nseg; }
+__host__ __device__ constexpr int sps_run_steps(const SpsGeom& g, int seg) { return sps_plane_lo(g.nplanes, seg + 1, g.nseg) - sps_plane_lo(g.nplanes, seg, g.nseg); }
+__host__ __device__ inline int sps_run_flagged(const SpsGeom& g, const unsigned char* sflags, int patch, int seg) {
+  int f = 0;
+  for (int pl = sps_plane_lo(g.nplanes, seg, g.nseg); pl < sps_plane_lo(g.nplanes, seg + 1, g.nseg); ++pl) f += sflags[(int64_t)pl * g.NP + patch] != 0;
+  return f;
+}
+__host__ __device__ inline int64_t sps_cost_of(const SpsGeom& g, const int32_t* flagged, int run) {
+  const int steps = sps_run_steps(g, run % g.nseg);
+  return sps_run_cost(steps - flagged[run], flagged[run]);
+}
+
+__host__ __device__ inline void sps_shares(const SpsGeom& g, const int32_t* flagged, int32_t* first) {
+  int64_t tot = 0, acc = 0;
+  for (int r = 0; r < sps_nruns(g); ++r) tot += sps_cost_of(g, flagged, r);
+  int k = 1;
+  first[0] = 0;
+  for (int p = 0; p < g.NP; ++p) {
+    for (int s = 0; s < g.nseg; ++s) acc += sps_cost_of(g, flagged, sps_run_id(p, s, g.nseg));
+    while (k < 8 && acc * 8 >= tot * k) first[k++] = p + 1;
+  }
+  while (k <= 8) first[k++] = g.NP;
+}
+__host__ __device__ constexpr uint64_t sps_mix(uint64_t z) {
+  z = (z ^ (z >> 30)) * 0xBF58476D1CE4E5B9ull;
+  z = (z ^ (z >> 27)) * 0x94D049BB133111EBull;
+  return z ^ (z >> 31);
+}
+__host__ __device__ inline uint64_t sps_list_key(const SpsGeom& g, const int32_t* flagged, int mode, uint64_t seed, int run) {
+  return mode == SPS_RANDOM ? sps_mix(~seed * 0x9E3779B97F4A7C15ull + (uint64_t)run) : (uint64_t)sps_cost_of(g, flagged, run);
+}
+
+__host__ __device__ inline void sps_build(const SpsGeom& g, const int32_t* flagged, int mode, uint64_t seed, int32_t* offset, int32_t* run, int32_t* first,
+                                          int64_t* load, int32_t* work) {
+  const int W = g.grid / 8, nruns = sps_nruns(g);
+  int32_t* wave_of = work;
+  int32_t* order = work + nruns;
+  int32_t* cursor = work + 2 * nruns;
+  for (int w = 0; w < g.grid; ++w) load[w] = 0;
+  for (int w = 0; w <= g.grid; ++w) offset[w] = 0;
+  if (mode == SPS_IDENTITY) {
+    for (int c = 0; c <= 8; ++c) first[c] = sps_eq_first(g.NP, c);
+    int n = 0;
+    for (int w = 0; w < g.grid; ++w) {
+      offset[w] = n;
+      for (int rk = 0; rk < sps_identity_rounds(g.NP, g.nseg, W, w & 7); ++rk) {
+        int patch = 0, seg = 0;
+        if (!sps_identity_run(g.NP, g.NPk, g.nseg, W, w & 7, w >> 3, rk, patch, seg)) continue;
+        run[n] = sps_run_id(patch, seg, g.nseg);
+        load[w] += sps_cost_of(g, flagged, run[n]);
+        ++n;
+      }
+    }
+    offset[g.grid] = n;
+    return;
+  }
+  sps_shares(g, flagged, first);
+  for (int c = 0; c < 8; ++c) {
+    const int r0 = first[c] * g.nseg, r1 = first[c + 1] * g.nseg, n = r1 - r0;
+    if (mode == SPS_RANDOM) {
+      for (int r = r0; r < r1; ++r) {
+        const int w = 8 * (int)(sps_mix(seed * 0x9E3779B97F4A7C15ull + (uint64_t)r + 1) % (uint64_t)W) + c;
+        wave_of[r] = w;
+        load[w] += sps_cost_of(g, flagged, r);
+      }
+      continue;
+    }
+    for (int i = 0; i < n; ++i) {
+      const int r = r0 + i;
+      const int64_t cr = sps_cost_of(g, flagged, r);
+      int j = i;
+      while (j > 0 && sps_cost_of(g, flagged, order[j - 1]) < cr) {
+        order[j] = order[j - 1];
+        --j;
+      }
+      order[j] = r;
+    }
+    for (int i = 0; i < n; ++i) {
+      int best = 0;
+      for (int jw = 1; jw < W; ++jw)
+        if (load[8 * jw + c] < load[8 * best + c]) best = jw;
+      wave_of[order[i]] = 8 * best + c;
+      load[8 * best + c] += sps_cost_of(g, flagged, order[i]);
+    }
+  }
+  for (int r = 0; r < nruns; ++r) ++offset[wave_of[r] + 1];
+  for (int w = 0; w < g.grid; ++w) {
+    offset[w + 1] += offset[w];
+    cursor[w] = offset[w];
+  }
+  for (int r = 0; r < nruns; ++r) run[cursor[wave_of[r]]++] = r;
+  for (int w = 0; w < g.grid; ++w)
+    for (int i = offset[w] + 1; i < offset[w + 1]; ++i) {
+      const int r = run[i];
+      const uint64_t kr = sps_list_key(g, flagged, mode, seed, r);
+      int j = i;
+      while (j > offset[w] && sps_list_key(g, flagged, mode, seed, run[j - 1]) < kr) {
+        run[j] = run[j - 1];
+        --j;
+      }
+      run[j] = r;
+    }
+}
+__host__ __device__ inline int64_t sps_makespan(const SpsGeom& g, const int64_t* load) {
+  int64_t m = 0;
+  for (int w = 0; w < g.grid; ++w) m = load[w] > m ? load[w] : m;
+  return m;
+}
```
